# terra-render/Terra

Hardware: AMD Instinct MI355X
Metric: Msamples/s (higher is better)
Workload: dtype f32; 1 GPU; cornell_1080p_512spp; scene=cornell32, width=1920, height=1080, spp=512, bounces=8, integrator=simple, triangles=32, tree=auto, traversal=reference tree + leaf-box cull, tile=64, sample_split=8, parallelism=single

## Files before the change

include/terra_amd.h:

```cpp
#ifndef TERRA_AMD_H
#define TERRA_AMD_H

#include "Terra.h"

#ifdef __cplusplus
extern "C" {
#endif

typedef enum {
    kTerraAmdOk               = 0,
    kTerraAmdErrNoDevice      = -1,
    kTerraAmdErrNotCommitted  = -2,
    kTerraAmdErrUnsupported   = -3,
    kTerraAmdErrBadArgument   = -4,
    kTerraAmdErrLaunch        = -5
} TerraAmdStatus;

const char* terra_amd_last_error ( void );
void        terra_amd_clear_error ( void );
int         terra_amd_first_error ( char* buf, size_t capacity );
void        terra_amd_clear_first_error ( void );
size_t      terra_amd_thread_staging_bytes ( void );

int  terra_amd_init ( void );
// ... 403 lines not shown
int terra_amd_sh_irradiance ( const TerraAmdProbeSH* sh, size_t probes, const TerraAmdProbeGrid* grid, const TerraAmdPoint* points, const int* index, size_t n, float* out4 );
int terra_amd_probe_grid_points ( const TerraAmdProbeGrid* grid, TerraAmdPoint* out, int capacity );

#define kTerraAmdProbeVisibilityBackface 1
typedef struct {
    int   texels;
    int   sharpness;
    float max_distance;
    float bias;
    int   flags;
    int   reserved[3];
} TerraAmdProbeVisibility;
typedef struct {
    float weight;
    float distance;
    float distance2;
    int   cells;
} TerraAmdVisibilityTexel;
TERRA_ABI_ASSERT ( sizeof ( TerraAmdProbeVisibility ) == 32 );
TERRA_ABI_ASSERT ( offsetof ( TerraAmdProbeVisibility, sharpness ) == 4 );
TERRA_ABI_ASSERT ( offsetof ( TerraAmdProbeVisibility, max_distance ) == 8 );
TERRA_ABI_ASSERT ( offsetof ( TerraAmdProbeVisibility, bias ) == 12 );
TERRA_ABI_ASSERT ( offsetof ( TerraAmdProbeVisibility, flags ) == 16 );
TERRA_ABI_ASSERT ( offsetof ( TerraAmdProbeVisibility, reserved ) == 20 );
TERRA_ABI_ASSERT ( sizeof ( TerraAmdVisibilityTexel ) == 16 );
TERRA_ABI_ASSERT ( offsetof ( TerraAmdVisibilityTexel, distance ) == 4 );
TERRA_ABI_ASSERT ( offsetof ( TerraAmdVisibilityTexel, distance2 ) == 8 );
TERRA_ABI_ASSERT ( offsetof ( TerraAmdVisibilityTexel, cells ) == 12 );
int terra_amd_probe_visibility_device ( const void* d_hits, const void* d_rays, size_t probes, int cells, const TerraAmdProbeVisibility* options, int accumulate, void* d_map, void* stream );
int terra_amd_probe_visibility ( const TerraAmdHit* hits, const TerraAmdRay* rays, size_t probes_n, int cells, const TerraAmdProbeVisibility* options, int accumulate, TerraAmdVisibilityTexel* map );
int terra_amd_sh_irradiance_visible_device ( const void* d_sh, const void* d_map, size_t probes, const TerraAmdProbeGrid* grid, const TerraAmdProbeVisibility* options, const void* d_points, size_t n, void* d_out, void* stream );
int terra_amd_sh_irradiance_visible ( const TerraAmdProbeSH* sh, const TerraAmdVisibilityTexel* map, size_t probes, const TerraAmdProbeGrid* grid, const TerraAmdProbeVisibility* options, const TerraAmdPoint* points, size_t n, float* out4 );

int terra_amd_render_device_sharded ( const TerraCamera* camera, HTerraScene scene,
                                      void* d_pixels, void* d_results, size_t fb_width, size_t fb_height,
                                      size_t x, size_t y, size_t width, size_t height,
                                      size_t tile_size, int rank, int world,
                                      void* d_rand_calls, void* stream );

int    terra_amd_shard_tile_count ( size_t width, size_t height, size_t tile_size, int rank, int world );
size_t terra_amd_shard_packed_bytes ( size_t width, size_t height, size_t tile_size, int world );
int terra_amd_pack_tiles ( const void* d_pixels, const void* d_results, size_t fb_width, size_t fb_height,
                           size_t x, size_t y, size_t width, size_t height, size_t tile_size, int rank, int world,
                           void* d_packed, void* stream );
int terra_amd_unpack_tiles ( void* d_pixels, void* d_results, size_t fb_width, size_t fb_height,
                             size_t x, size_t y, size_t width, size_t height, size_t tile_size, int rank, int world,
                             const void* d_packed, void* stream );

int terra_amd_synchronize ( void* stream );

int terra_amd_time_render_device ( const TerraCamera* camera, HTerraScene scene,
                                   void* d_pixels, void* d_results, size_t fb_width, size_t fb_height,
                                   size_t x, size_t y, size_t width, size_t height,
                                   int launches, void* stream, float* ms_avg );


int terra_amd_unit_pcg ( const uint32_t* seeds, int nseeds, int n, float* out );
int terra_amd_unit_stream_keys ( uint64_t frame_seed, const uint64_t* pix, const uint64_t* samples_so_far, int n, uint64_t* out3 );
int terra_amd_unit_ray_aabb ( int n, const float* origins3, const float* dirs3, const float* boxes6, int* hit, float* tmin, float* tmax );
int terra_amd_unit_watertight ( int n, const float* origins3, const float* dirs3, const float* tris9, int* hit, float* out8 );
int terra_amd_unit_watertight_pair ( int n, const float* origins3, const float* dirs3, const float* quads12, int* hit2, float* depth2 );
int terra_amd_unit_moller_trumbore ( int n, const float* origins3, const float* dirs3, const float* tris9, int* hit, float* out4 );
int terra_amd_unit_bvh_traverse ( HTerraScene scene, int n, const float* origins3, const float* dirs3, int* found, uint32_t* prim, float* point3 );
int terra_amd_unit_bvh_traverse_fast ( HTerraScene scene, int n, const float* origins3, const float* dirs3, int* found, uint32_t* prim, float* point3, uint32_t* nodes_visited );
int terra_amd_unit_raycast ( HTerraScene scene, int n, const float* origins3, const float* dirs3, int* obj, int* tri, float* point3, float* surface47 );
int terra_amd_unit_trace ( HTerraScene scene, int n, const float* origins3, const float* dirs3, const uint64_t* stateB, const uint64_t* incB, float* radiance3, uint32_t* rand_calls );
int terra_amd_unit_bsdf ( int kind, int n, float* surfaces47, const float* e3, const float* wo3, float* wi3, float* pdf, float* f3 );
int terra_amd_unit_bsdf_at ( int kind, int n, const float* surfaces47, const float* wi3, const float* wo3, float* pdf, float* f3 );
int terra_amd_unit_camera ( const TerraCamera* camera, size_t fb_width, size_t fb_height, int n, const uint32_t* xy2, float jitter, const float* r2, float* dirs3 );
int terra_amd_unit_tonemap ( int op, float gamma, int n, float* colors3 );
int terra_amd_unit_math ( int fn, int n, const float* x, const float* y, float* out );
int terra_amd_scene_lds_plan ( HTerraScene scene, uint32_t* out6 );
int terra_amd_unit_exact_div ( int op, const float* a, const float* b, const float* c, uint64_t first, uint64_t count, float denominator, float reciprocal, uint64_t seed,
                               uint32_t* helper_bits, uint32_t* plain_bits, uint64_t* mismatches, uint32_t* first_bad );
int terra_amd_unit_exact_sqrt ( int op, const float* a, const float* b, const float* c, uint64_t first, uint64_t count, uint64_t seed,
                                uint32_t* helper_bits, uint32_t* plain_bits, uint64_t* mismatches, uint32_t* first_bad );
int terra_amd_unit_half_outward ( const double* x, int n, int up, uint16_t* out );
int terra_amd_unit_stratified ( const uint32_t* seeds, int nseeds, int strata, int samples_per_stratum, int n, float* out2 );
int terra_amd_unit_halton ( int first, int n, float* out2 );
int terra_amd_unit_distribution_1d ( const float* f, size_t n, const float* e, int m, float* x, float* pdf, uint32_t* idx, float* cdf_out, float* integral_out );
int terra_amd_unit_distribution_2d ( const float* f, size_t nx, size_t ny, const float* e12, int m, float* xy2, float* pdf, float* marginal_cdf_out );
int terra_amd_unit_distribution_2d_pdf ( const float* f, size_t nx, size_t ny, const float* xy2, int m, float* pdf );
int terra_amd_unit_azimuth24 ( uint32_t* mismatches );
int terra_amd_unit_texture_sample ( const TerraTexture* texture, int n, const float* uv2, float* out3 );
int terra_amd_unit_texture_latlong ( const TerraTexture* texture, int n, const float* dir3, float* out3 );

#ifdef __cplusplus
}
#endif
#endif
```

terra_amd/csrc/dev_types.h:

```cpp
#pragma once
#include <stdint.h>
#include <stddef.h>
#include <hip/hip_vector_types.h>

#define TERRA_DEV_MAX_ATTR 8

struct DevF3 { float x, y, z; };
struct DevF4 { float x, y, z, w; };

#define DEV_CHILD_LEAF  0x80000000u
#define DEV_CHILD_EMPTY 0xFFFFFFFFu

struct DevNode {
    float    min0[3], max0[3];
    float    min1[3], max1[3];
    uint32_t child[2];
    uint32_t prim[2];
};
static_assert ( sizeof ( DevNode ) == 64, "DevNode must be 64 bytes" );

struct DevFastNode {
    uint32_t q[3][2][4];
    uint32_t child[4];
    uint32_t pad[4];
// ... 104 lines not shown
#define TERRA_LEAF_CAP_RESIDENT_MIN 8
#endif
#ifndef TERRA_LDS_BLOCK_MAX_KB
#define TERRA_LDS_BLOCK_MAX_KB 156
#endif
#ifndef TERRA_JOB_ORDER_MIN_BLOCKS
#define TERRA_JOB_ORDER_MIN_BLOCKS 256
#endif

struct DevScene {
    const DevNode*     nodes;
    const DevTri*      tris;
    const DevProps*    props;
    const DevMaterial* mats;
    const DevLight*    lights;
    const float*       tri_area;
    const DevTexture*  textures;
    uint32_t n_nodes, n_tris, n_objects, n_lights;
    uint32_t lights_triangles_count;
    int32_t  max_stack;
    const DevNode*     fast_nodes;
    const DevFastNode* fast_nodes_h;
    const DevTri*      fast_tris;
    uint32_t n_fast_nodes;
    int32_t  fast_max_stack;
    float    fast_inv_scale;
    const struct DevReplay* ref_replay;
    const uint32_t*    fast_leaf_parent;
    const uint32_t*    fast_leaf_mask;
    uint32_t           reach;
    const float2*      sincos24;
    int32_t  env_mode;
    int32_t  env_tex;
    float    env_color[3];
    const float* env_f; const float* env_cdf; const float* env_row_f; const float* env_row_cdf;
    uint32_t env_nx, env_ny; float env_integral; uint32_t env_monotone;
};
#define TERRA_KIND_ENV 16
#define TERRA_KIND_TEX 32
#define TERRA_KIND_SAMPLER 64
#define TERRA_KIND_ENV_MIS 128

enum { kCtrRays = 0, kCtrNodes, kCtrBoxTests, kCtrTriTests, kCtrHits, kCtrSamples, kCtrRandCalls, kCtrAttrFetches, kCtrPixels, kCtrLaunches, kCtrFaults, kCtrTriCulled,
       kCtrDbg0, kCtrDbgLast = kCtrDbg0 + 15, kCtrSkipProved , kCtrCount };

struct DevRenderParams {
    DevScene scene;
    float    cam_rot[9];
    float    cam_pos[3];
    float    tan_half_fov;
    float    aspect;
    float    jitter;
    float    exposure;
    float    gamma;
    uint32_t fb_w, fb_h;
    uint32_t x, y, w, h;
    uint32_t st_x, st_y, st_pitch;
    uint32_t tile_size, rank, world;
    uint32_t spp;
    uint32_t split, split_log2, chunk_spp;
    float4*  partials;
    uint4*   job_streams;
    uint32_t job_blocks;
    uint32_t* job_queue;
    const uint32_t* block_order;
    uint32_t job_div_bpt2, job_div_tiles_x, job_div_bpt, job_tiles_x;
    uint32_t bounces;
    int32_t  integrator;
    int32_t  tonemap;
    uint64_t frame_seed;
    float*   pixels;
    void*    results;
    uint32_t* rand_calls;
    unsigned long long* counters;
    uint32_t stack_depth, leaf_cap, lds_nodes, lds_tris;
    uint32_t* stack_spill; uint32_t spill_cap;
    int32_t  lds_mode;
    int32_t  count_level;
    uint32_t bsdf_kinds;
    uint32_t leaf_cull;
    uint32_t fused_slab;
    uint32_t leaf_rank;
    uint32_t sampler_mode, sampler_strata;
    const uint32_t* job_live;
    const DevLeafBox* leaf_boxes;
    uint32_t n_leaf_boxes;
    uint32_t leaf_pairs;
    float    inv_fb_w, inv_fb_h;
};
struct DevLaunchMask { const uint32_t* words; uint32_t* live_blocks; };
#define TERRA_CLASS_MASKED 3u
struct DevRayRenderParams : DevRenderParams { const float4* rays; };
struct DevLens {
    int32_t model;
    float   lens_radius;
    float   focus_distance;
    float   ortho_half;
    float   fisheye_half;
};
struct DevLensRenderParams : DevRenderParams { DevLens lens; };
struct DevPointSampling {
    int32_t distribution;
};
struct DevPointRenderParams : DevRenderParams { const float4* points; DevPointSampling sampling; };
#ifndef TERRA_RAY_SOURCE
#if defined ( TERRA_TU ) && TERRA_TU >= 12
#define TERRA_RAY_SOURCE 3
#elif defined ( TERRA_TU ) && TERRA_TU >= 8
#define TERRA_RAY_SOURCE 2
#elif defined ( TERRA_TU ) && TERRA_TU >= 4
#define TERRA_RAY_SOURCE 1
#else
#define TERRA_RAY_SOURCE 0
#endif
#endif
```

terra_amd/csrc/exact_div.h:

```cpp
#pragma once
#include <hip/hip_runtime.h>
#include <stdint.h>

#define XD __device__ __forceinline__

XD int xd_in_range ( float v ) { const float a = __builtin_fabsf ( v ); return ( int ) ( a >= 0x1p-60f ) & ( int ) ( a <= 0x1p60f ); }
XD int xd_rcp_ok ( float d ) { return xd_in_range ( d ) & ( int ) ( ( __float_as_uint ( d ) & 0x7fffffu ) != 0x7fffffu ); }

XD float xd_rcp_short ( float d ) {
    float y = __builtin_amdgcn_rcpf ( d );
    float e = __builtin_fmaf ( -d, y, 1.f );
    y = __builtin_fmaf ( e, y, y );
    e = __builtin_fmaf ( -d, y, 1.f );
    return __builtin_fmaf ( e, y, y );
}
XD float xd_div_short ( float x, float d, float r ) {
    const float q0 = x * r;
    const float rem = __builtin_fmaf ( -d, q0, x );
    return __builtin_fmaf ( rem, r, q0 );
}
XD float xd_div_short_pos ( float x, float d, float r ) {
    const float q0 = x * r;
    const float nrem = __builtin_fmaf ( d, q0, -x );
    return __builtin_fmaf ( -nrem, r, q0 );
}

XD float rcp_exact ( float d ) {
    if ( xd_rcp_ok ( d ) ) return xd_rcp_short ( d );
    return 1.f / d;
}
XD float div_exact_r ( float x, float d, float r ) {
    if ( xd_in_range ( x ) & xd_in_range ( d ) ) return xd_div_short ( x, d, r );
    return x / d;
}
XD float div_exact_rk ( float x, float d, float r ) {
    if ( xd_in_range ( x ) ) return xd_div_short ( x, d, r );
    return x / d;
}
XD void div2_exact_rk ( float x1, float x2, float d1, float r1, float d2, float r2, float& q1, float& q2 ) {
    if ( xd_in_range ( x1 ) & xd_in_range ( x2 ) ) { q1 = xd_div_short ( x1, d1, r1 ); q2 = xd_div_short ( x2, d2, r2 ); return; }
    q1 = x1 / d1; q2 = x2 / d2;
}
XD void div2_exact ( float x1, float x2, float d, float& q1, float& q2 ) {
    if ( xd_rcp_ok ( d ) & xd_in_range ( x1 ) & xd_in_range ( x2 ) ) {
        const float r = xd_rcp_short ( d );
        q1 = xd_div_short ( x1, d, r ); q2 = xd_div_short ( x2, d, r );
        return;
    }
    q1 = x1 / d; q2 = x2 / d;
}
XD void rcp3_exact ( float dx, float dy, float dz, float& rx, float& ry, float& rz ) {
    if ( xd_rcp_ok ( dx ) & xd_rcp_ok ( dy ) & xd_rcp_ok ( dz ) ) { rx = xd_rcp_short ( dx ); ry = xd_rcp_short ( dy ); rz = xd_rcp_short ( dz ); return; }
    rx = 1.f / dx; ry = 1.f / dy; rz = 1.f / dz;
}
XD int xd_component_ok ( float c ) { return ( int ) ( c == 0.f ) | ( int ) ( __builtin_fabsf ( c ) >= 0x1p-60f ); }
XD void xd_normalize3 ( float x, float y, float z, float l, float& qx, float& qy, float& qz ) {
    if ( ( int ) ( l >= 0x1p-60f ) & ( int ) ( l <= 0x1p60f ) & ( int ) ( ( __float_as_uint ( l ) & 0x7fffffu ) != 0x7fffffu ) & xd_component_ok ( x ) & xd_component_ok ( y ) & xd_component_ok ( z ) ) {
        const float r = xd_rcp_short ( l );
        qx = xd_div_short_pos ( x, l, r ); qy = xd_div_short_pos ( y, l, r ); qz = xd_div_short_pos ( z, l, r );
        return;
    }
    qx = x / l; qy = y / l; qz = z / l;
}

XD float roulette_scale ( float pr ) {
    const double d = ( double ) pr + 1e-4;
    if ( ( int ) ( pr >= 0.f ) & ( int ) ( pr <= 0x1p60f ) ) {
        double y = __builtin_amdgcn_rcp ( d );
        double e = __builtin_fma ( -d, y, 1.0 ); y = __builtin_fma ( y, e, y );
        e = __builtin_fma ( -d, y, 1.0 ); y = __builtin_fma ( y, e, y );
        e = __builtin_fma ( -d, y, 1.0 ); y = __builtin_fma ( e, y, y );
        return ( float ) y;
    }
    return ( float ) ( 1.0 / d );
}
```

terra_amd/csrc/exact_sqrt.h:

```cpp
#pragma once
#include <hip/hip_runtime.h>
#include <stdint.h>
#include "exact_div.h"

XD float xs_sqrt_short ( float x ) {
    const float s = __builtin_amdgcn_sqrtf ( x );
    const float down = __uint_as_float ( __float_as_uint ( s ) - 1u ), up = __uint_as_float ( __float_as_uint ( s ) + 1u );
    const float r_down = __builtin_fmaf ( -down, s, x ), r_up = __builtin_fmaf ( -up, s, x );
    float r = r_down <= 0.f ? down : s;
    r = r_up > 0.f ? up : r;
    return r;
}
XD int xs_in_range ( float x ) { return ( int ) ( x >= 0x1p-96f ) & ( int ) ( x <= 0x1.fffffep127f ); }
XD float sqrt_exact ( float x ) {
    if ( xs_in_range ( x ) ) return xs_sqrt_short ( x );
    return sqrtf ( x );
}
```

terra_amd/csrc/integrators_device.h:

```cpp
#pragma once
#include "shading_device.h"

TD float randf ( Pcg32& b, Counters& c, int count ) { if ( count == 2 ) ++c.rand_calls; return trng_b_float ( b ); }
TD uint32_t randf_bits ( Pcg32& b, Counters& c, int count ) { if ( count == 2 ) ++c.rand_calls; return trng_b_bits ( b ); }

TD float triangle_area ( V3 a, V3 b, V3 cc ) { return length ( cross ( b - a, cc - a ) ) / 2; }

struct LightSample { uint32_t light_object; uint32_t tri_in_object; uint32_t tri; float pick_pdf; V3 pos, norm; };

template <int COUNT, int MODE = 0>
TD LightSample draw_light_sample ( const DevScene& sc, Pcg32& rb, Counters& c, const Tracer* T = nullptr ) {
    LightSample ls;
    float e = ( float ) ( ( double ) randf ( rb, c, COUNT ) - 1e-4 );
    double xl = ( double ) e * ( double ) sc.n_lights;
    uint32_t li = xl < 0 ? 0u : ( uint32_t ) xl;
    ls.pick_pdf = 1.f / ( float ) sc.lights_triangles_count;
    DevLight l = ( MODE == 1 && T ) ? T->l_lights[li] : sc.lights[li];
    float e_t = randf ( rb, c, COUNT );
    uint32_t k = ( uint32_t ) ( e_t * ( float ) l.tri_count );
    if ( k >= l.tri_count ) k = l.tri_count - 1;
    ls.light_object = l.object; ls.tri_in_object = k; ls.tri = l.first_tri + k;
    float e1 = randf ( rb, c, COUNT ), e2 = randf ( rb, c, COUNT );
    const float4* tris = ( MODE == 1 && T ) ? reinterpret_cast<const float4*> ( T->l_tris ) : reinterpret_cast<const float4*> ( sc.tris );
    const float4* props = ( MODE == 1 && T ) ? T->l_props : reinterpret_cast<const float4*> ( sc.props );
// ... 236 lines not shown
                    L = L * ( dot ( wi, sf.normal ) * weight / bpdf );
                    Lo = Lo + L;
                }
            }
        }
        if constexpr ( ( KINDS & TERRA_KIND_ENV_MIS ) != 0 && !DEBUG_WEIGHTS ) {
            if ( !h.hit && bpdf > 0.f ) {
                uint32_t col, row; float st;
                environment_texel ( sc, wi, col, row, st );
                const float epdf = ( !bsdf_is_singular<KINDS> ( sf ) && dot ( wi, sf.normal ) > 0 ) ? environment_texel_pdf ( sc, col, row, st ) : 0.f;
                const float r = epdf / bpdf, weight = 1.f / ( 1.f + r * r );
                V3 L = had ( texture_read ( sc.textures[sc.env_tex], col, row ), f );
                L = L * ( dot ( wi, sf.normal ) * weight / bpdf );
                Lo = Lo + L;
            }
        }
    }
    if constexpr ( ( KINDS & TERRA_KIND_SAMPLER ) != 0 && !DEBUG_WEIGHTS ) { if ( env_sampling_active ( sc ) ) Lo = Lo + environment_light_sample<COUNT, MODE, KINDS, true> ( T, sf, p, wo, rb, c ); }
    return had ( Lo, throughput );
}

TD V3 integrate_debug_normals ( const Surface& sf, uint32_t bounce ) {
    if ( bounce != 0 ) return v3 ( 0, 0, 0 );
    V3 n = sf.normal;
    V3 pp = v3 ( sel_min ( n.x > 0 ? n.x : 0.f, 1.f ), sel_min ( n.y > 0 ? n.y : 0.f, 1.f ), sel_min ( n.z > 0 ? n.z : 0.f, 1.f ) );
    V3 nn = v3 ( sel_min ( n.x > -1 ? n.x : -1.f, 0.f ), sel_min ( n.y > -1 ? n.y : -1.f, 0.f ), sel_min ( n.z > -1 ? n.z : -1.f, 0.f ) );
    nn = nn * -1.f;
    V3 col = v3 ( 0, 0, 0 );
    col = col + v3 ( 1, 0, 0 ) * pp.x;
    col = col + v3 ( 0, 1, 0 ) * pp.y;
    col = col + v3 ( 0, 0, 1 ) * pp.z;
    col = col + v3 ( 0, 1, 1 ) * nn.x;
    col = col + v3 ( 1, 0, 1 ) * nn.y;
    col = col + v3 ( 1, 1, 0 ) * nn.z;
    return col;
}

template <int INTEGRATOR, int COUNT, int MODE, int KINDS>
TD V3 integrate ( const Tracer& T, const Ray& ray, Surface& sf, V3 p, V3 wo, V3 throughput, uint32_t bounce, Pcg32& rb, Counters& c ) {
    if ( INTEGRATOR == 0 ) {
        if ( dot ( wo, sf.normal ) > 0 ) return had ( sf.emissive, throughput );
        return v3 ( 0, 0, 0 );
    } else if ( INTEGRATOR == 1 ) {
        return integrate_direct<COUNT, MODE, KINDS> ( T, sf, p, wo, throughput, bounce, rb, c );
    } else if ( INTEGRATOR == 2 ) {
        return integrate_mis<COUNT, MODE, KINDS, false> ( T, sf, p, wo, throughput, bounce, rb, c );
    } else if ( INTEGRATOR == 3 ) {
        return bounce != 0 ? v3 ( 0, 0, 0 ) : v3 ( 1, 1, 1 );
    } else if ( INTEGRATOR == 4 ) {
        if ( bounce != 0 ) return v3 ( 0, 0, 0 );
        float d = length ( ray.o - p ) / 500.f;
        return v3 ( d, d, d );
    } else if ( INTEGRATOR == 5 ) {
        return integrate_debug_normals ( sf, bounce );
    } else {
        return integrate_mis<COUNT, MODE, KINDS, true> ( T, sf, p, wo, throughput, bounce, rb, c );
    }
}

template <int COUNT>
TD PathDraws path_draw ( const float2* sincos24, Pcg32& rb, Counters& c ) {
    PathDraws d;
    d.e0 = randf ( rb, c, COUNT );
    const uint32_t k1 = randf_bits ( rb, c, COUNT );
    d.e1 = trng_b_from_bits ( k1 );
    d.e2 = randf ( rb, c, COUNT );
    d.az = azimuth_fetch_index ( sincos24, k1 );
    d.e3 = randf ( rb, c, COUNT );
    return d;
}
template <int KINDS>
TD bool path_continue ( Surface& sf, V3 wo, V3& throughput, uint32_t& bounce, uint32_t max_bounces, const PathDraws& d, V3& wi ) {
    wi = bsdf_sample<KINDS> ( sf, d.e0, d.e1, d.e2, wo, d.az );
    float pdf = sel_max ( bsdf_pdf<KINDS> ( sf, wi, wo ), ( float ) 1e-4 );
    V3 f = bsdf_eval<KINDS> ( sf, wi, wo ) * rcp_exact ( pdf );
    throughput = had ( throughput, f );
    throughput = throughput * dot ( sf.normal, wi );
    float pr = sel_max ( throughput.x, sel_max ( throughput.y, throughput.z ) );
    if ( d.e3 > pr ) return false;
        throughput = throughput * roulette_scale ( pr );
    ++bounce;
    return bounce <= max_bounces;
}
struct SamplerPair { float u0, u1; bool on; };
TD SamplerPair sampler_pair_none() { SamplerPair s; s.u0 = s.u1 = 0.f; s.on = false; return s; }
TD void path_apply_sampler ( PathDraws& d, const SamplerPair& sp, uint32_t bounce ) {
    if ( sp.on && bounce == 0 ) { d.e0 = sp.u0; d.e1 = sp.u1; d.az = azimuth_none(); }
}
TD SamplerPair sampler_pair_draw ( uint32_t mode, uint32_t strata, uint64_t n, Pcg32& stream_a ) {
    SamplerPair s = sampler_pair_none();
    if ( mode == 1 ) { s.u0 = radical_inverse ( 3, n ); s.u1 = radical_inverse ( 2, n ); s.on = true; }
    else if ( mode == 2 && strata > 0 ) {
        const uint64_t cap = ( uint64_t ) strata * strata * 16ull, m = n % cap, stratum = m / 16ull;
        const float stratum_size = 1.f / ( float ) strata;
        s.u0 = sd_below_one ( ( ( float ) ( uint32_t ) ( stratum % strata ) + trng_a_float ( stream_a ) ) * stratum_size );
        s.u1 = sd_below_one ( ( ( float ) ( uint32_t ) ( stratum / strata ) + trng_a_float ( stream_a ) ) * stratum_size );
        s.on = true;
    }
    return s;
}
template <int COUNT, int KINDS>
TD bool path_continue ( const DevScene& sc, Surface& sf, V3 wo, V3& throughput, uint32_t& bounce, uint32_t max_bounces, Pcg32& rb, Counters& c, V3& wi, const SamplerPair& sp = sampler_pair_none() ) {
    PathDraws d = path_draw<COUNT> ( sc.sincos24, rb, c );
    if ( KINDS & TERRA_KIND_SAMPLER ) path_apply_sampler ( d, sp, bounce );
    return path_continue<KINDS> ( sf, wo, throughput, bounce, max_bounces, d, wi );
}

template <int INTEGRATOR, int COUNT, int MODE, int KINDS>
TD V3 trace_path ( const Tracer& T, Ray ray, uint32_t bounces, Pcg32& rb, Counters& c ) {
    V3 Lo = v3 ( 0, 0, 0 ), throughput = v3 ( 1, 1, 1 );
    for ( uint32_t bounce = 0; bounce <= bounces; ++bounce ) {
        Surface sf;
        RaycastResult h = scene_raycast<COUNT, MODE, KINDS> ( T, ray, sf, c );
        if ( !h.hit ) {
            if ( ( KINDS & TERRA_KIND_ENV ) && T.sc.env_mode && !env_reaches_by_samples<INTEGRATOR, KINDS> ( T.sc, bounce ) ) { throughput = had ( throughput, environment_eval ( T.sc, ray.d ) ); Lo = Lo + throughput; }
            break;
        }
        V3 wo = neg ( ray.d );
        Lo = Lo + integrate<INTEGRATOR, COUNT, MODE, KINDS> ( T, ray, sf, h.point, wo, throughput, bounce, rb, c );
        V3 wi;
        uint32_t next_bounce = bounce;
        if ( !path_continue<COUNT, KINDS> ( T.sc, sf, wo, throughput, next_bounce, bounces, rb, c, wi ) ) break;
        ray = surface_ray ( sf, h.point, wi );
    }
    return Lo;
}

TD V3 uncharted2 ( V3 x ) {
    const float A = 0.15f, B = 0.5f, C = 0.1f, D = 0.2f, E = 0.02f, F = 0.3f;
    V3 r;
    r.x = ( ( x.x * ( A * x.x + C * B ) + D * E ) / ( x.x * ( A * x.x + B ) + D * F ) ) - E / F;
    r.y = ( ( x.y * ( A * x.y + C * B ) + D * E ) / ( x.y * ( A * x.y + B ) + D * F ) ) - E / F;
    r.z = ( ( x.z * ( A * x.z + C * B ) + D * E ) / ( x.z * ( A * x.z + B ) + D * F ) ) - E / F;
    return r;
}
TD V3 powv ( V3 c, float e ) { return v3 ( tdm_powf ( c.x, e ), tdm_powf ( c.y, e ), tdm_powf ( c.z, e ) ); }
TD V3 tonemap ( V3 c, int op, float gamma ) {
    switch ( op ) {
        case 1: c = powv ( c, 1.f / gamma ); break;
        case 2:
            c.x = c.x / ( 1.f + c.x ); c.y = c.y / ( 1.f + c.y ); c.z = c.z / ( 1.f + c.z );
            c = powv ( c, 1.f / gamma ); break;
        case 3: {
            V3 x = v3 ( sel_max ( 0.f, c.x - 0.004f ), sel_max ( 0.f, c.y - 0.004f ), sel_max ( 0.f, c.z - 0.004f ) );
            c.x = ( x.x * ( 6.2f * x.x + 0.5f ) ) / ( x.x * ( 6.2f * x.x + 1.7f ) + 0.06f );
            c.y = ( x.y * ( 6.2f * x.y + 0.5f ) ) / ( x.y * ( 6.2f * x.y + 1.7f ) + 0.06f );
            c.x = ( x.z * ( 6.2f * x.z + 0.5f ) ) / ( x.z * ( 6.2f * x.z + 1.7f ) + 0.06f );
            break;
        }
        case 4: {
            V3 ws = uncharted2 ( v3 ( 11.2f, 11.2f, 11.2f ) );
            ws = v3 ( 1.f / ws.x, 1.f / ws.y, 1.f / ws.z );
            V3 t = uncharted2 ( c * 2.f );
            c = powv ( had ( t, ws ), 1.f / gamma );
            break;
        }
        default: break;
    }
    return c;
}
```

terra_amd/csrc/kernels.h:

```cpp
#pragma once
#include <hip/hip_runtime.h>
#include "dev_types.h"

hipError_t terra_launch_render ( const DevRenderParams& p, hipStream_t stream );
hipError_t terra_launch_job_streams ( const DevRenderParams& p, hipStream_t stream );
hipError_t terra_launch_block_order ( const DevRenderParams& p, uint32_t* cls, hipStream_t stream, const DevLaunchMask* mask, bool classify, bool prove );
hipError_t terra_launch_render_mode0 ( const DevRenderParams& p, size_t lds, hipStream_t stream );
hipError_t terra_launch_render_mode1 ( const DevRenderParams& p, size_t lds, hipStream_t stream );
hipError_t terra_launch_render_mode2 ( const DevRenderParams& p, size_t lds, hipStream_t stream );
hipError_t terra_launch_render_mode3 ( const DevRenderParams& p, size_t lds, hipStream_t stream );
hipError_t terra_launch_render_rays ( const DevRenderParams& p, const void* rays, hipStream_t stream );
hipError_t terra_launch_render_rays_mode0 ( const DevRayRenderParams& p, size_t lds, hipStream_t stream );
hipError_t terra_launch_render_rays_mode1 ( const DevRayRenderParams& p, size_t lds, hipStream_t stream );
hipError_t terra_launch_render_rays_mode2 ( const DevRayRenderParams& p, size_t lds, hipStream_t stream );
hipError_t terra_launch_render_rays_mode3 ( const DevRayRenderParams& p, size_t lds, hipStream_t stream );
hipError_t terra_launch_render_lens ( const DevRenderParams& p, const DevLens& lens, hipStream_t stream );
hipError_t terra_launch_render_lens_mode0 ( const DevLensRenderParams& p, size_t lds, hipStream_t stream );
hipError_t terra_launch_render_lens_mode1 ( const DevLensRenderParams& p, size_t lds, hipStream_t stream );
hipError_t terra_launch_render_lens_mode2 ( const DevLensRenderParams& p, size_t lds, hipStream_t stream );
hipError_t terra_launch_render_lens_mode3 ( const DevLensRenderParams& p, size_t lds, hipStream_t stream );
hipError_t terra_launch_render_points ( const DevRenderParams& p, const void* points, const DevPointSampling& sampling, hipStream_t stream );
hipError_t terra_launch_render_points_mode0 ( const DevPointRenderParams& p, size_t lds, hipStream_t stream );
hipError_t terra_launch_render_points_mode1 ( const DevPointRenderParams& p, size_t lds, hipStream_t stream );
hipError_t terra_launch_render_points_mode2 ( const DevPointRenderParams& p, size_t lds, hipStream_t stream );
hipError_t terra_launch_render_points_mode3 ( const DevPointRenderParams& p, size_t lds, hipStream_t stream );
hipError_t terra_launch_resolve ( const DevRenderParams& p, hipStream_t stream, const uint32_t* live_blocks );
hipError_t terra_launch_tiles ( bool pack, float* pixels, void* results, uint32_t fb_w, uint32_t x, uint32_t y, uint32_t w, uint32_t h,
                                uint32_t tile, uint32_t rank, uint32_t world, float* packed, hipStream_t stream );

hipError_t terra_launch_aov ( DevRenderParams p, void* aov, hipStream_t stream, const uint32_t* mask );
hipError_t terra_launch_aov_rays ( DevRenderParams p, const void* rays, void* aov, hipStream_t stream );
hipError_t terra_launch_aov_lens ( DevRenderParams p, const DevLens& lens, void* aov, hipStream_t stream );
hipError_t terra_launch_aov_points ( DevRenderParams p, const void* points, const DevPointSampling& sampling, void* aov, hipStream_t stream );

hipError_t terra_launch_denoise ( const void* results, const void* aov, uint32_t fb_w, uint32_t x, uint32_t y, uint32_t w, uint32_t h, int iterations,
                                  float exposure, int op, float gamma, float* radiance, float* pixels, hipStream_t stream );
hipError_t terra_launch_denoise_variance ( const void* results, const void* aov, const void* moments, uint32_t fb_w, uint32_t x, uint32_t y, uint32_t w, uint32_t h, int iterations,
                                           float exposure, int op, float gamma, float* radiance, float* pixels, hipStream_t stream );

hipError_t terra_launch_moments_accumulate ( const void* results, void* moments, uint32_t fb_w, uint32_t x, uint32_t y, uint32_t w, uint32_t h, hipStream_t stream );
hipError_t terra_launch_tile_error ( const void* moments, uint32_t fb_w, uint32_t x, uint32_t y, uint32_t w, uint32_t h, uint32_t tile, float* errors, hipStream_t stream );
hipError_t terra_launch_error_mask ( const float* errors, uint32_t w, uint32_t h, uint32_t tile, float target, int all, uint32_t* mask, hipStream_t stream );

struct DevTemporalParams {
    float cam_pos[3], cam_rot[9], tan_half_fov, aspect;
    float prev_pos[3], prev_rot[9], prev_tan_half_fov;
    uint32_t fb_w, fb_h, x, y, w, h;
    float alpha, depth_tolerance, normal_cos, max_length;
    uint32_t same_camera;
    float inv_fb_w, inv_fb_h;
};
hipError_t terra_launch_temporal_reproject ( const DevTemporalParams& p, const void* results, const void* aov, const void* history_in, void* history_out,
                                             void* out_results, void* out_moments, hipStream_t stream );

struct DevQueryParams {
    DevScene scene;
    uint32_t fast, stack_depth, leaf_cap, spill_cap, leaf_cull;
    float    origin_limit;
};
hipError_t terra_launch_query ( DevQueryParams p, const void* rays, size_t n, void* out, bool anyhit, hipStream_t stream );

struct DevAtlas {
    uint32_t width, height;
    float    uv_scale[2], uv_offset[2], margin;
};
hipError_t terra_launch_atlas_points ( const DevScene& sc, const DevAtlas& atlas, const float* uvs, void* points, void* texels, hipStream_t stream );
hipError_t terra_launch_dilate ( float* data, int channels, int* valid, uint32_t width, uint32_t height, int passes, hipStream_t stream );

struct DevProbeGrid {
    int32_t on;
    int32_t count[3];
    float   origin[3], spacing[3];
};
hipError_t terra_launch_probe_rays ( const void* probes, uint32_t count, uint32_t cells, const float* jitter, void* rays, hipStream_t stream );
hipError_t terra_launch_sh_project ( const void* results, const void* rays, uint32_t count, uint32_t cells, int batch, void* sh, hipStream_t stream );
hipError_t terra_launch_sh_irradiance ( const void* sh, uint32_t probes, const DevProbeGrid& grid, const void* points, const int* index, uint32_t n, void* out, hipStream_t stream );
struct DevProbeVisibility {
    int32_t texels, sharpness;
    float   max_distance, bias;
    int32_t backface;
};
hipError_t terra_launch_probe_visibility ( const void* hits, const void* rays, uint32_t count, uint32_t cells, const DevProbeVisibility& options, int accumulate, void* map, hipStream_t stream );
hipError_t terra_launch_sh_irradiance_visible ( const void* sh, const void* map, const DevProbeGrid& grid, const DevProbeVisibility& options, const void* points, uint32_t n, void* out, hipStream_t stream );

hipError_t terra_fill_sincos24 ( float2* table, hipStream_t stream );
hipError_t terra_unit_azimuth24 ( const float2* table, float2* computed, uint32_t* mismatches );

hipError_t terra_unit_pcg ( const uint32_t* seeds, int nseeds, int n, float* out );
hipError_t terra_unit_stream_keys ( uint64_t frame_seed, const uint64_t* pix, const uint64_t* k, int n, uint64_t* out3 );
hipError_t terra_unit_ray_aabb ( int n, const float* o, const float* d, const float* boxes, int* hit, float* tmin, float* tmax );
hipError_t terra_unit_watertight ( int n, const float* o, const float* d, const float* tris, int* hit, float* out8 );
hipError_t terra_unit_watertight_pair ( int n, const float* o, const float* d, const float* quads, int* hit, float* depth );
hipError_t terra_unit_moller_trumbore ( int n, const float* o, const float* d, const float* tris, int* hit, float* out4 );
hipError_t terra_unit_bvh_traverse ( const DevScene& sc, int n, const float* o, const float* d, int* found, uint32_t* prim, float* point );
hipError_t terra_unit_bvh_traverse_fast ( const DevScene& sc, int n, const float* o, const float* d, int* found, uint32_t* prim, float* point, uint32_t* nodes_visited );
hipError_t terra_unit_raycast ( const DevScene& sc, int n, const float* o, const float* d, int* obj, int* tri, float* point, float* surface47 );
hipError_t terra_unit_trace ( const DevScene& sc, int integrator, uint32_t bounces, int n, const float* o, const float* d,
                              const uint64_t* stateB, const uint64_t* incB, float* radiance, uint32_t* rand_calls );
hipError_t terra_unit_bsdf ( int kind, int n, float* surfaces47, const float* e3, const float* wo3, float* wi3, float* pdf, float* f3 );
hipError_t terra_unit_bsdf_at ( int kind, int n, const float* surfaces47, const float* wi3, const float* wo3, float* pdf, float* f3 );
hipError_t terra_unit_camera ( const DevRenderParams& p, int n, const uint32_t* xy2, const float* r2, float* dirs3 );
hipError_t terra_unit_lens_rays ( const DevRenderParams& p, const DevLens& lens, int n, const uint32_t* xy2, const float* r4, float* rays8 );
hipError_t terra_unit_point_rays ( const DevPointSampling& sampling, int n, const float* points8, const float* g2, float* rays8 );
hipError_t terra_unit_tonemap ( int op, float gamma, int n, float* colors3 );
hipError_t terra_unit_math ( int fn, int n, const float* x, const float* y, float* out );
hipError_t terra_unit_exact_div ( int op, const float* a, const float* b, const float* c, uint64_t first, uint64_t count, float D, float R, uint64_t seed,
                                  uint32_t* helper_bits, uint32_t* plain_bits, unsigned long long* mismatches, uint32_t* first_bad );
hipError_t terra_unit_exact_sqrt ( int op, const float* a, const float* b, const float* c, uint64_t first, uint64_t count, uint64_t seed,
                                   uint32_t* helper_bits, uint32_t* plain_bits, unsigned long long* mismatches, uint32_t* first_bad );
hipError_t terra_unit_texture_sample ( const DevTexture* t, int n, const float* uv2, float* out3 );
hipError_t terra_unit_texture_latlong ( const DevTexture* t, int n, const float* dir3, float* out3 );
hipError_t terra_unit_stratified ( const uint32_t* seeds, int nseeds, int strata, int samples, int n, float* out2 );
hipError_t terra_unit_halton ( int first, int n, float* out2 );
hipError_t terra_unit_distribution_1d ( const float* f, uint32_t n, float* cdf, float* integral, uint32_t* monotone, const float* e, int m, float* x, float* pdf, uint32_t* idx );
hipError_t terra_unit_distribution_2d ( const float* f, uint32_t nx, uint32_t ny, float* cdf, float* integrals, float* mcdf, uint32_t* monotone, const float* e12, int m, float* xy2, float* pdf );
hipError_t terra_unit_distribution_2d_pdf ( const float* f, uint32_t nx, uint32_t ny, float* cdf, float* integrals, float* mcdf, uint32_t* monotone, const float* xy2, int m, float* pdf );
hipError_t terra_build_fast_tree_device ( const DevTri* tris, const uint32_t* rank, uint32_t n, float extra_margin, DevNode* out_nodes, DevTri* out_tris, uint32_t* n_nodes_out, int* max_stack_out, hipStream_t stream );
```

terra_amd/csrc/render_kernels.hip:

```cpp
#include <hip/hip_runtime.h>
#include "trace_device.h"
#include "kernels.h"
#include "launch_plan.h"
#include "empty_proof.h"

#ifdef TERRA_TU
#define TERRA_TU_HAS(k) ( TERRA_TU == ( k ) )
#define TERRA_TU_MODE(k) ( TERRA_TU == ( k ) || TERRA_TU == ( k ) + 4 || TERRA_TU == ( k ) + 8 || TERRA_TU == ( k ) + 12 )
#else
#define TERRA_TU_HAS(k) ( !TERRA_RAY_SOURCE )
#define TERRA_TU_MODE(k) 1
#endif
#if TERRA_RAY_SOURCE == 3
typedef DevPointRenderParams RenderKernelParams;
#elif TERRA_RAY_SOURCE == 2
typedef DevLensRenderParams RenderKernelParams;
#elif TERRA_RAY_SOURCE == 1
typedef DevRayRenderParams RenderKernelParams;
#else
typedef DevRenderParams RenderKernelParams;
#endif

struct DevResult { float acc[3]; int samples; };

// ... 322 lines not shown
        p.partials[ ( ( size_t ) chunk * ( p.job_blocks >> p.split_log2 ) + blk ) * 256 + ( fin & 255u )] = make_float4 ( aux[0], aux[256], aux[512], __uint_as_float ( COUNT == 2 ? c.rand_calls - auxu[1024] : 0u ) );
        auxu[768] = TERRA_JOB_NONE;
    }
    PoolWord* pool = job_pool_of_wave ( aux );
    const unsigned long long m = __ballot ( 1 );
    const uint32_t lane = threadIdx.x & 63u, n = ( uint32_t ) __popcll ( m ), ahead = ( uint32_t ) __popcll ( m & ( ( 1ull << lane ) - 1ull ) );
    uint32_t next = pool_load ( pool ), end = pool_load ( pool + 1 );
    const uint32_t take = n < end - next ? n : end - next;
    uint32_t job = next + ahead;
    bool got = ahead < take;
    next += take;
    if ( take < n && next < total && p.job_queue ) {
        uint32_t base = 0;
        if ( ahead == 0 ) base = atomicAdd ( p.job_queue, TERRA_JOB_BATCH );
        base = ( uint32_t ) __builtin_amdgcn_readfirstlane ( ( int ) base );
        next = base < total ? base : total; end = base + TERRA_JOB_BATCH < total ? base + TERRA_JOB_BATCH : total;
        const uint32_t take2 = n - take < end - next ? n - take : end - next;
        if ( !got ) { job = next + ( ahead - take ); got = ahead - take < take2; }
        next += take2;
    }
    if ( ahead == 0 ) { pool_store ( pool, next ); pool_store ( pool + 1, end ); }
    if ( !got ) { j.exhausted = true; return; }
    uint32_t chunk;
    int prior_samples;
    if constexpr ( TABLE ) {
        const uint4 e1 = p.job_streams[2 * ( size_t ) job + 1];
        const uint4 e0 = p.job_streams[2 * ( size_t ) job];
        asm volatile ( "" : : "v" ( e0.x ), "v" ( e0.y ), "v" ( e0.z ), "v" ( e0.w ), "v" ( e1.x ), "v" ( e1.y ), "v" ( e1.z ), "v" ( e1.w ) );
        if ( e1.z == 0xffffffffu ) return;
        j.px = e1.z & 0xffffu; j.py = e1.z >> 16;
        chunk = ( job >> 8 ) & ( p.split - 1 );
        rs.a.state = ( uint64_t ) e0.x | ( ( uint64_t ) e0.y << 32 ); rs.a.inc = 1;
        rs.b.state = ( uint64_t ) e0.z | ( ( uint64_t ) e0.w << 32 ); rs.b.inc = ( uint64_t ) e1.x | ( ( uint64_t ) e1.y << 32 );
        rs.seedA = 0;
        prior_samples = ( int ) e1.w;
    } else {
        if ( !job_pixel ( p, job, j.px, j.py, chunk ) ) return;
        prior_samples = reinterpret_cast<const DevResult*> ( p.results ) [ ( size_t ) ( j.py - p.st_y ) * p.st_pitch + ( j.px - p.st_x )].samples;
        rs = trng_pixel_streams ( p.frame_seed, ( uint64_t ) j.py * p.fb_w + j.px, ( uint64_t ) ( uint32_t ) prior_samples + ( uint64_t ) chunk * p.chunk_spp );
    }
    aux[0] = 0.f; aux[256] = 0.f; aux[512] = 0.f; auxu[768] = job;
    if ( COUNT == 2 ) auxu[1024] = c.rand_calls;
    j.s = 0; j.base = ( uint32_t ) prior_samples + chunk * p.chunk_spp;
}

#ifndef TERRA_RAY_HOLD
#define TERRA_RAY_HOLD 0
#endif
struct PrimaryRay { V3 o, d; };
TD PrimaryRay ray_record ( const RenderKernelParams& p, uint32_t px, uint32_t py ) {
    PrimaryRay r; r.o = v3 ( 0, 0, 0 ); r.d = v3 ( 0, 0, 1 );
#if TERRA_RAY_SOURCE == 1
    const float4* rec = p.rays + 2 * ( ( size_t ) ( py - p.st_y ) * p.st_pitch + ( px - p.st_x ) );
    const float4 q0 = rec[0], q1 = rec[1];
    r.o = v3 ( q0.x, q0.y, q0.z ); r.d = v3 ( q1.x, q1.y, q1.z );
#elif TERRA_RAY_SOURCE == 3
    const float4* rec = p.points + 2 * ( ( size_t ) ( py - p.st_y ) * p.st_pitch + ( px - p.st_x ) );
    const float4 q0 = rec[0], q1 = rec[1];
    r.o = v3 ( q0.x, q0.y, q0.z ); r.d = v3 ( q1.x, q1.y, q1.z );
#endif
    return r;
}
TD bool ray_record_inactive ( const PrimaryRay& r ) {
    const bool finite = fabsf ( r.o.x ) < INFINITY && fabsf ( r.o.y ) < INFINITY && fabsf ( r.o.z ) < INFINITY && fabsf ( r.d.x ) < INFINITY && fabsf ( r.d.y ) < INFINITY && fabsf ( r.d.z ) < INFINITY;
    return !finite || ( r.d.x == 0.f && r.d.y == 0.f && r.d.z == 0.f );
}
#ifndef TERRA_POINT_HOLD
#define TERRA_POINT_HOLD 0
#endif
#if TERRA_RAY_SOURCE == 3
#define TERRA_PRIMARY_RAY( ro, rd, r1, r2 )
#define TERRA_LENS_RAY( ro, rd, r1, r2 ) do { const PrimaryRay pt_ = TERRA_POINT_HOLD ? held : ray_record ( p, jb.px, jb.py ); const float g1_ = trng_a_float ( rs.a ), g2_ = trng_a_float ( rs.a ); point_sample ( p.sampling, pt_.o, pt_.d, g1_, g2_, ro, rd ); } while ( 0 )
#define TERRA_JOB_NEXT() job_take<COUNT, MODE == 1> ( p, acc_lds, jb, rs, c, job_total, held )
#elif TERRA_RAY_SOURCE == 2
#define TERRA_PRIMARY_RAY( ro, rd, r1, r2 )
#define TERRA_LENS_RAY( ro, rd, r1, r2 ) do { float l1_ = 0.f, l2_ = 0.f; if ( lens_draws ( p.lens ) ) { l1_ = trng_a_float ( rs.a ); l2_ = trng_a_float ( rs.a ); } lens_sample ( p, p.lens, jb.px, jb.py, r1, r2, l1_, l2_, ro, rd ); } while ( 0 )
#define TERRA_JOB_NEXT() job_next<COUNT, MODE == 1> ( p, acc_lds, jb, rs, c, job_total )
#elif TERRA_RAY_SOURCE == 1
#define TERRA_PRIMARY_RAY( ro, rd, r1, r2 ) do { const PrimaryRay pr_ = TERRA_RAY_HOLD ? held : ray_record ( p, jb.px, jb.py ); ro = pr_.o; rd = pr_.d; } while ( 0 )
#define TERRA_LENS_RAY( ro, rd, r1, r2 )
#define TERRA_JOB_NEXT() job_take<COUNT, MODE == 1> ( p, acc_lds, jb, rs, c, job_total, held )
#else
#define TERRA_LENS_RAY( ro, rd, r1, r2 )
#define TERRA_PRIMARY_RAY( ro, rd, r1, r2 ) ro = cam_pos; rd = camera_sample ( p, jb.px, jb.py, r1, r2 )
#define TERRA_JOB_NEXT() job_next<COUNT, MODE == 1> ( p, acc_lds, jb, rs, c, job_total )
#endif
#if TERRA_RAY_SOURCE == 1 || TERRA_RAY_SOURCE == 3
template <int COUNT, bool TABLE>
TD void job_take ( const RenderKernelParams& p, float* aux, Jobs& j, PixelStreams& rs, const Counters& c, uint32_t total, PrimaryRay& held ) {
    job_next<COUNT, TABLE> ( p, aux, j, rs, c, total );
    if ( j.s != p.chunk_spp ) {
        const PrimaryRay r = ray_record ( p, j.px, j.py );
#if TERRA_RAY_SOURCE == 3
        if ( point_inactive ( r.o, r.d ) ) j.s = p.chunk_spp;
        if ( TERRA_POINT_HOLD ) held = r;
#else
        if ( ray_record_inactive ( r ) ) j.s = p.chunk_spp;
        if ( TERRA_RAY_HOLD ) held = r;
#endif
    }
}
#endif

template <int INTEGRATOR, int COUNT, int MODE, int KINDS>
__global__ __launch_bounds__ ( 256, terra_waves ( INTEGRATOR, KINDS, MODE ) ) void terra_render_kernel ( RenderKernelParams p ) {
    extern __shared__ float4 lds_f4[];
    const int tid = threadIdx.x;
    Tracer T0 = make_tracer<MODE> ( p.scene, lds_f4, p.stack_depth, p.leaf_cap, p.lds_nodes, p.lds_tris, p.leaf_cull != 0, p.fused_slab != 0, p.leaf_rank != 0, p.leaf_boxes, p.n_leaf_boxes, terra_leaf_pair_table ( p ) );
    if constexpr ( MODE == 1 && COUNT == 0 ) T0.nearest = T0.pairs && T0.n_boxes != 0u && ( p.leaf_pairs & TERRA_LEAF_PAIRS_NEAREST ) != 0u;
    T0.faults = p.counters + kCtrFaults;
    if ( MODE >= 2 && p.stack_spill ) { T0.spill = p.stack_spill + ( size_t ) ( blockIdx.x * 256u + threadIdx.x ) * p.spill_cap; T0.spill_cap = p.spill_cap; }
    const Tracer T = T0;

    PixelStreams rs = trng_pixel_streams ( 0, 0, 0 );
    Counters c = counters_zero();
    float* acc_lds = reinterpret_cast<float*> ( T.stack - tid ) + ( p.stack_depth + p.leaf_cap ) * TERRA_COL + tid;
    uint32_t job_total = p.job_blocks * 256u;
    if constexpr ( MODE == 1 ) { if ( p.job_live ) job_total = *p.job_live; }
    job_init_lane ( p, acc_lds );
    Jobs jb; jb.px = jb.py = 0; jb.s = p.chunk_spp; jb.exhausted = false; jb.base = 0;
    SamplerPair sp = sampler_pair_none();
    V3 Lo = v3 ( 0, 0, 0 ), throughput = v3 ( 1, 1, 1 );
    Ray ray = make_ray ( v3 ( 0, 0, 0 ), v3 ( 0, 0, 1 ) );
    uint32_t bounce = 0;
    const V3 cam_pos = v3p ( p.cam_pos );
#if TERRA_RAY_SOURCE == 1 || TERRA_RAY_SOURCE == 3
    PrimaryRay held; held.o = v3 ( 0, 0, 0 ); held.d = v3 ( 0, 0, 1 );
#endif

    if constexpr ( terra_decoupled_mis ( INTEGRATOR, MODE, KINDS ) ) {
        LaneTraversal lt = lane_traversal_idle ( T, ray );
        int job = 0;
        bool done = false, have_ray = false, cont = false;
        MisPending pend; pend.a_vis = pend.a_hid = pend.f2 = pend.p = pend.t_before = v3 ( 0, 0, 0 ); pend.expected = 0; pend.bpdf2 = pend.cos2 = 0.f; pend.light_object = 0;
        V3 cont_o = v3 ( 0, 0, 0 ), cont_d = v3 ( 0, 0, 1 ), b_o = v3 ( 0, 0, 0 ), b_d = v3 ( 0, 0, 1 ), lo_i = v3 ( 0, 0, 0 );
        for ( ;; ) {
            if ( !lt.traversing && !done && ! ( have_ray && lane_traversal_recheck<MODE> ( T, ray, lt ) ) ) {
                bool start = false;
                V3 ro = v3 ( 0, 0, 0 ), rd = v3 ( 0, 0, 1 );
                if ( have_ray && job != 0 ) {
                    Ray r = ray; r.o = r.o + r.d * 0.001f;
                    const bool hit = lt.best.tri != 0xffffffffu;
                    Surface lsf; uint32_t object = 0, tri_in_object = 0, nattr = 0, tri_s = 0xffffffffu;
                    V3 point = hit ? r.o + r.d * lt.best.depth : v3 ( FLT_MAX, FLT_MAX, FLT_MAX );
                    if ( hit ) {
                        if ( job == 2 ) { surface_init<MODE, KINDS> ( T, lt.best.tri, point, lsf, object, tri_in_object, nattr ); tri_s = MODE >= 2 ? T.sc.mats[object].first_tri + tri_in_object : lt.best.tri; }
                        else { tri_s = hit_soup_index<MODE> ( T, lt.best.tri ); const float4 t0 = reinterpret_cast<const float4*> ( T.sc.tris ) [3 * tri_s]; object = __float_as_uint ( t0.w ); nattr = T.sc.mats[object].attributes_count; }
                        if ( COUNT ) ++c.hits;
                        if ( COUNT == 2 ) c.attr_fetches += nattr + 1;
                    }
                    if ( job == 1 ) {
                        lo_i = tri_s == pend.expected ? pend.a_vis : pend.a_hid;
                        ro = b_o; rd = b_d; job = 2; start = true;
                    } else {
                        Lo = Lo + mis_finish_b<MODE> ( T, pend, lo_i, hit, object, tri_s, point, lsf, ray.d );
                        job = 0;
                        if ( cont ) { ro = cont_o; rd = cont_d; start = true; }
                        else { deposit ( acc_lds, Lo ); have_ray = false; }
                    }
                } else if ( have_ray ) {
                    if ( lt.best.tri != 0xffffffffu ) {
                        Surface sf;
                        V3 point = shade_surface<COUNT, MODE, KINDS> ( T, ray, lt.best, sf, c );
                        V3 wo = neg ( ray.d );
                        Ray ray_a;
                        pend = mis_prepare<COUNT, KINDS, MODE> ( T, sf, point, wo, throughput, bounce, rs.b, c, ray_a, b_d );
                        b_o = surface_origin ( sf, point );
// ... 57 lines not shown
                    if ( jb.s == p.chunk_spp ) { TERRA_JOB_NEXT(); if ( jb.exhausted ) done = true; }
                    if ( jb.s != p.chunk_spp ) {
                        float r1 = trng_a_float ( rs.a ), r2 = trng_a_float ( rs.a );
                        TERRA_PRIMARY_RAY ( ro, rd, r1, r2 );
                        if constexpr ( ( KINDS & TERRA_KIND_SAMPLER ) != 0 ) sp = sampler_pair_draw ( p.sampler_mode, p.sampler_strata, ( uint64_t ) jb.base + jb.s, rs.a );
                        TERRA_LENS_RAY ( ro, rd, r1, r2 );
                        Lo = v3 ( 0, 0, 0 ); throughput = v3 ( 1, 1, 1 ); bounce = 0; ++jb.s; start = true;
                    }
                }
                if ( start ) {
                    ray = make_ray ( ro, rd ); lane_traversal_start<COUNT, MODE> ( T, ray, lt, c ); have_ray = true;
                    if ( shadow ) lane_traversal_expect<COUNT, MODE> ( T, ray, lt, pend.expected );
                }
            }
            if ( !lane_traversal_run<COUNT, MODE> ( T, ray, lt, c ) && __all ( done ) ) break;
        }
    } else if constexpr ( terra_decoupled ( INTEGRATOR, MODE ) ) {
        LaneTraversal lt = lane_traversal_idle ( T, ray );
        bool done = false, have_ray = false;
        for ( ;; ) {
            if ( !lt.traversing && !done && ! ( have_ray && lane_traversal_recheck<MODE> ( T, ray, lt ) ) ) {
                bool next = false;
                V3 ro = v3 ( 0, 0, 0 ), rd = v3 ( 0, 0, 1 );
                if ( have_ray ) {
                    if ( lt.best.tri != 0xffffffffu ) {
                        Surface sf;
                        PathDraws pd = path_draw<COUNT> ( azimuth_table<MODE> ( T.sc ), rs.b, c );
                        if constexpr ( ( KINDS & TERRA_KIND_SAMPLER ) != 0 ) path_apply_sampler ( pd, sp, bounce );
                        V3 point = shade_surface<COUNT, MODE, KINDS> ( T, ray, lt.best, sf, c );
                        V3 wo = neg ( ray.d ), wi;
                        Lo = Lo + integrate<INTEGRATOR, COUNT, MODE, KINDS> ( T, ray, sf, point, wo, throughput, bounce, rs.b, c );
                        next = path_continue<KINDS> ( sf, wo, throughput, bounce, p.bounces, pd, wi );
                        if ( next ) { ro = surface_origin ( sf, point ); rd = wi; }
                    } else if ( ( KINDS & TERRA_KIND_ENV ) && T.sc.env_mode ) {
                        throughput = had ( throughput, environment_eval ( T.sc, ray.d ) );
                        Lo = Lo + throughput;
                    }
                    if ( !next ) { deposit ( acc_lds, Lo ); have_ray = false; }
                }
                if ( !next ) {
                    if ( jb.s == p.chunk_spp ) { TERRA_JOB_NEXT(); if ( jb.exhausted ) done = true; }
                    if ( jb.s != p.chunk_spp ) {
                        float r1 = trng_a_float ( rs.a ), r2 = trng_a_float ( rs.a );
                        TERRA_PRIMARY_RAY ( ro, rd, r1, r2 );
                        if constexpr ( ( KINDS & TERRA_KIND_SAMPLER ) != 0 ) sp = sampler_pair_draw ( p.sampler_mode, p.sampler_strata, ( uint64_t ) jb.base + jb.s, rs.a );
                        TERRA_LENS_RAY ( ro, rd, r1, r2 );
                        Lo = v3 ( 0, 0, 0 ); throughput = v3 ( 1, 1, 1 ); bounce = 0; ++jb.s; next = true;
                    }
                }
                if ( next ) { ray = make_ray ( ro, rd ); lane_traversal_start<COUNT, MODE> ( T, ray, lt, c ); have_ray = true; }
            }
            if ( !lane_traversal_run<COUNT, MODE> ( T, ray, lt, c ) && __all ( done ) ) break;
        }
    } else {
    bool alive = false;
    V3 ro = v3 ( 0, 0, 0 ), rd = v3 ( 0, 0, 1 );
    constexpr bool LO_LDS = MODE == 1;
    float* lo_lds = acc_lds + 6 * 256;
    auto lo_reset = [&] () { if ( LO_LDS ) { lo_lds[0] = 0.f; lo_lds[256] = 0.f; lo_lds[512] = 0.f; } else Lo = v3 ( 0, 0, 0 ); };
    auto lo_add = [&] ( V3 t ) {
        if ( LO_LDS ) { if ( t.x != 0.f || t.y != 0.f || t.z != 0.f ) { lo_lds[0] = lo_lds[0] + t.x; lo_lds[256] = lo_lds[256] + t.y; lo_lds[512] = lo_lds[512] + t.z; } }
        else Lo = Lo + t;
    };
    auto lo_deposit = [&] () { if ( LO_LDS ) deposit ( acc_lds, v3 ( lo_lds[0], lo_lds[256], lo_lds[512] ) ); else deposit ( acc_lds, Lo ); };
#ifndef TERRA_REGEN_MIN
#define TERRA_REGEN_MIN 1
#endif
    while ( true ) {
        const bool any_alive = __any ( alive );
        if ( !alive && ( TERRA_REGEN_MIN <= 1 || !any_alive || __popcll ( __ballot ( !alive ) ) >= TERRA_REGEN_MIN ) ) {
            if ( jb.s == p.chunk_spp && ( TERRA_JOB_FETCH_MIN <= 1 || !any_alive || __popcll ( __ballot ( jb.s == p.chunk_spp ) ) >= TERRA_JOB_FETCH_MIN ) ) TERRA_JOB_NEXT();
            if ( jb.exhausted ) break;
            if ( jb.s != p.chunk_spp ) {
                PS_WAVE ( c, kPsCamIter ); PS_LANE ( c, kPsCamLanes );
                float r1 = trng_a_float ( rs.a ), r2 = trng_a_float ( rs.a );
                TERRA_PRIMARY_RAY ( ro, rd, r1, r2 );
                if constexpr ( ( KINDS & TERRA_KIND_SAMPLER ) != 0 ) sp = sampler_pair_draw ( p.sampler_mode, p.sampler_strata, ( uint64_t ) jb.base + jb.s, rs.a );
                TERRA_LENS_RAY ( ro, rd, r1, r2 );
                lo_reset(); throughput = v3 ( 1, 1, 1 ); bounce = 0; alive = true; ++jb.s;
            }
        }
        if ( alive ) {
            bool guarded = false;
            if constexpr ( ray_start_masks_for ( COUNT, MODE, KINDS ) ) ray = make_ray_guarded ( ro, rd, guarded ); else
            ray = make_ray ( ro, rd );
            Surface sf;
            PS_WAVE ( c, kPsRayIter ); PS_LANE ( c, kPsRayLanes );
            constexpr bool pre_draw = !TERRA_IS_LIGHT ( INTEGRATOR );
            PathDraws pd;
            RaycastResult h = scene_raycast<COUNT, MODE, KINDS> ( T, ray, sf, c, pre_draw ? &pd : nullptr, pre_draw ? &rs.b : nullptr, guarded );
            bool end = !h.hit;
            if ( h.hit ) {
                PS_WAVE ( c, kPsShadeIter ); PS_LANE ( c, kPsShadeLanes );
                V3 wo = neg ( ray.d ), wi;
                constexpr bool SPLIT_DIRECT = INTEGRATOR == 1 && ( KINDS & ( TERRA_KIND_TEX | TERRA_KIND_SAMPLER ) ) == 0;
                if constexpr ( SPLIT_DIRECT ) {
                    Ray shadow_ray;
                    const DirectPending pend = direct_prepare<COUNT, KINDS, MODE> ( T, sf, h.point, wo, throughput, bounce, rs.b, c, shadow_ray );
                    pd = path_draw<COUNT> ( azimuth_table<MODE> ( T.sc ), rs.b, c );
                    end = !path_continue<KINDS> ( sf, wo, throughput, bounce, p.bounces, pd, wi );
                    if ( !end ) { ro = surface_origin ( sf, h.point ); rd = wi; }
                    const uint32_t tri = scene_raycast_triangle<COUNT, MODE, ray_start_masks_for ( COUNT, MODE, KINDS )> ( T, shadow_ray, c, pend.expected );
                    lo_add ( tri == pend.expected ? pend.vis : pend.hid );
                } else if constexpr ( INTEGRATOR == 2 && ( KINDS & ( TERRA_KIND_TEX | TERRA_KIND_SAMPLER ) ) == 0 ) {
                    Ray ray_a; V3 b_d;
                    const MisPending pend = mis_prepare<COUNT, KINDS, MODE> ( T, sf, h.point, wo, throughput, bounce, rs.b, c, ray_a, b_d );
                    const V3 next_o = surface_origin ( sf, h.point );
                    end = !path_continue<COUNT, KINDS> ( T.sc, sf, wo, throughput, bounce, p.bounces, rs.b, c, wi, sp );
                    if ( !end ) { ro = next_o; rd = wi; }
                    const uint32_t tri_a = scene_raycast_triangle<COUNT, MODE, ray_start_masks_for ( COUNT, MODE, KINDS )> ( T, ray_a, c, pend.expected );
                    const V3 lo_a = tri_a == pend.expected ? pend.a_vis : pend.a_hid;
                    Surface lsf;
                    const RaycastResult hb = scene_raycast<COUNT, MODE, KINDS> ( T, make_ray ( next_o, b_d ), lsf, c );
                    lo_add ( mis_finish_b<MODE> ( T, pend, lo_a, hb.hit, hb.object, hb.tri, hb.point, lsf, b_d ) );
                } else {
                lo_add ( integrate<INTEGRATOR, COUNT, MODE, KINDS> ( T, ray, sf, h.point, wo, throughput, bounce, rs.b, c ) );
                if ( !pre_draw ) pd = path_draw<COUNT> ( azimuth_table<MODE> ( T.sc ), rs.b, c );
                if constexpr ( ( KINDS & TERRA_KIND_SAMPLER ) != 0 ) path_apply_sampler ( pd, sp, bounce );
                end = !path_continue<KINDS> ( sf, wo, throughput, bounce, p.bounces, pd, wi );
                if ( !end ) { ro = surface_origin ( sf, h.point ); rd = wi; }
                }
            } else if ( ( KINDS & TERRA_KIND_ENV ) && T.sc.env_mode && !env_reaches_by_samples<INTEGRATOR, KINDS> ( T.sc, bounce ) ) {
                throughput = had ( throughput, environment_eval ( T.sc, ray.d ) );
                lo_add ( throughput );
            }
            if ( end ) { lo_deposit(); alive = false; }
        }
    }
    }

    if ( COUNT ) wave_flush_counters ( c, p.counters );
    if ( COUNT == 2 && p.leaf_cull ) {
        unsigned long long x = c.tri_culled;
        for ( int off = 32; off > 0; off >>= 1 ) x += __shfl_xor ( x, off, 64 );
        if ( ( threadIdx.x & 63 ) == 0 && x ) atomicAdd ( &p.counters[kCtrTriCulled], x );
    }
#if TERRA_PHASE_STATS
    for ( int k = 0; k < 16; ++k ) {
        unsigned long long x = c.ps[k];
        for ( int off = 32; off > 0; off >>= 1 ) x += __shfl_xor ( x, off, 64 );
        if ( ( threadIdx.x & 63 ) == 0 && x ) atomicAdd ( &p.counters[kCtrDbg0 + k], x );
    }
#endif
}


static uint32_t resident_blocks ( const void* fn, size_t lds ) {
    struct Key { const void* fn; size_t lds; int dev; uint32_t blocks; };
    static thread_local Key cache[8]; static thread_local int used = 0;
    int dev = 0; ( void ) hipGetDevice ( &dev );
    for ( int i = 0; i < used; ++i ) if ( cache[i].fn == fn && cache[i].lds == lds && cache[i].dev == dev ) return cache[i].blocks;
    int per_cu = 0;
    if ( hipOccupancyMaxActiveBlocksPerMultiprocessor ( &per_cu, fn, 256, lds ) != hipSuccess || per_cu < 1 ) { ( void ) hipGetLastError(); per_cu = 1; }
    const uint32_t blocks = ( uint32_t ) per_cu * terra_cu_count();
    Key& k = cache[used < 8 ? used++ : 7]; k.fn = fn; k.lds = lds; k.dev = dev; k.blocks = blocks;
    return blocks;
}
template <int I, int COUNT, int MODE, int KINDS>
static hipError_t launch_instance ( const RenderKernelParams& p, size_t lds, hipStream_t stream ) {
    auto fn = terra_render_kernel<I, COUNT, MODE, KINDS>;
    if ( lds > ( size_t ) 64 * 1024 ) {
        if ( lds > terra_lds_block_limit() ) return hipErrorInvalidValue;
        static thread_local size_t opted[8] = { 0 }; int dev = 0; ( void ) hipGetDevice ( &dev );
        if ( opted[dev & 7] < lds ) {
            const hipError_t e = hipFuncSetAttribute ( reinterpret_cast<const void*> ( fn ), hipFuncAttributeMaxDynamicSharedMemorySize, ( int ) lds );
            if ( e != hipSuccess ) return e;
            opted[dev & 7] = lds;
        }
    }
    uint32_t grid = p.job_blocks;
    if ( p.job_queue ) { const uint32_t cap = resident_blocks ( reinterpret_cast<const void*> ( fn ), lds ); if ( grid > cap ) grid = cap; }
    if ( MODE >= 2 && p.spill_cap && ( !p.stack_spill || terra_spill_bytes ( grid, p.spill_cap ) > terra_fast_spill_bytes ( p ) ) ) return hipErrorInvalidValue;
    hipLaunchKernelGGL ( fn, dim3 ( grid ), dim3 ( 256 ), lds, stream, p );
    return hipGetLastError();
}
template <int I, int MODE, int KINDS>
static hipError_t launch_kinds ( const RenderKernelParams& p, size_t lds, hipStream_t stream ) {
    if ( p.count_level == 0 ) return launch_instance<I, 0, MODE, KINDS> ( p, lds, stream );
    return launch_instance<I, 2, MODE, KINDS> ( p, lds, stream );
}
template <int I, int MODE>
static hipError_t launch_mode ( const RenderKernelParams& p, size_t lds, hipStream_t stream ) {
    if ( p.bsdf_kinds == 1 ) return launch_kinds<I, MODE, 1> ( p, lds, stream );
    if ( ( p.bsdf_kinds & ~3u ) == 0 ) return launch_kinds<I, MODE, 3> ( p, lds, stream );
    if constexpr ( I <= 2 && MODE != 0 ) {
        if ( ( p.bsdf_kinds & ~15u ) == 0 ) return launch_kinds<I, MODE, 15> ( p, lds, stream );
    }
    if ( ( p.bsdf_kinds & TERRA_KIND_SAMPLER ) == 0 ) return launch_kinds<I, MODE, TERRA_KINDS_ALL & ~TERRA_KIND_SAMPLER> ( p, lds, stream );
    if constexpr ( I == 2 ) {
        if ( p.bsdf_kinds & TERRA_KIND_ENV_MIS ) return launch_kinds<I, MODE, TERRA_KINDS_ALL | TERRA_KIND_ENV_MIS> ( p, lds, stream );
    }
    return launch_kinds<I, MODE, TERRA_KINDS_ALL> ( p, lds, stream );
}
template <int MODE>
static hipError_t launch_integrator ( const RenderKernelParams& p, size_t lds, hipStream_t stream ) {
    switch ( p.integrator ) {
        case 0: return launch_mode<0, MODE> ( p, lds, stream );
        case 1: return launch_mode<1, MODE> ( p, lds, stream );
        case 2: return launch_mode<2, MODE> ( p, lds, stream );
        case 3: return launch_mode<3, MODE> ( p, lds, stream );
        case 4: return launch_mode<4, MODE> ( p, lds, stream );
// ... 251 lines not shown
```

terra_amd/csrc/scene_host.cpp:

```cpp
#include <hip/hip_runtime.h>
#include <algorithm>
#include <cfloat>
#include <cmath>
#include <cstdarg>
#include <cstdio>
#include <cstdlib>
#include <cstring>
#include <mutex>
#include <string>
#include <unordered_set>
#include <atomic>
#include <chrono>
#include <vector>

#include "../../include/terra_amd.h"
#include "../../include/TerraPresets.h"
#include "dev_types.h"
#include "kernels.h"
#include "launch_plan.h"
#include "empty_proof.h"
#include "tree_build.h"
#include "multi_gpu.h"

static thread_local std::string g_last_error;
// ... 1240 lines not shown
    out6[3] = ( uint32_t ) TERRA_LDS_BUDGET; out6[4] = p.lds_mode == 1 ? p.lds_tris : 0u; out6[5] = p.leaf_rank;
    return 0;
}
extern "C" int terra_amd_leaf_pair_offsets ( uint32_t n, uint32_t* entries, uint32_t* planes ) {
    if ( n > TERRA_LEAF_RANK_MAX / 2 ) return fail ( kTerraAmdErrBadArgument, "terra_amd_leaf_pair_offsets: a pair section has at most %u entries", ( unsigned ) TERRA_LEAF_RANK_MAX / 2 );
    for ( uint32_t perm = 0; perm < 6u && entries; ++perm ) for ( uint32_t e = 0; e < n; ++e ) entries[perm * n + e] = terra_pair_entry_offset ( n, perm, e );
    for ( uint32_t k = 0; k < n && planes; ++k ) for ( uint32_t as = 0; as < 6u; ++as ) planes[6u * k + as] = terra_pair_boxes_offset ( n ) + terra_pair_box_plane_offset ( k, as >> 1, as & 1u );
    return ( int ) terra_pair_section_bytes ( n );
}
extern "C" int terra_amd_leaf_box_offsets ( uint32_t n, uint32_t* planes, uint32_t* masks ) {
    if ( n > TERRA_LEAF_RANK_MAX ) return fail ( kTerraAmdErrBadArgument, "terra_amd_leaf_box_offsets: a table has at most %u boxes", ( unsigned ) TERRA_LEAF_RANK_MAX );
    for ( uint32_t k = 0; k < n; ++k ) {
        for ( uint32_t as = 0; as < 6u && planes; ++as ) planes[6u * k + as] = terra_leaf_box_plane_offset ( k, as >> 1, as & 1u );
        if ( masks ) masks[k] = terra_leaf_box_mask_offset ( k );
    }
    return n ? ( int ) ( terra_leaf_box_plane_offset ( n - 1u, 0, 0 ) - terra_leaf_box_plane_offset ( 0, 0, 0 ) ) : 0;
}
static int sum_counters ( Scene* s, size_t first, size_t n, unsigned long long* out ) {
    unsigned long long c[kCtrCount];
    std::fill ( out, out + n, 0ull );
    for ( size_t k = s->replicas.size(); k-- > 0; ) {
        const Scene::Replica& r = s->replicas[k];
        HIP_TRY ( hipSetDevice ( r.device ), kTerraAmdErrNoDevice );
        HIP_TRY ( hipMemcpy ( c, r.d_counters + first, n * sizeof ( unsigned long long ), hipMemcpyDeviceToHost ), kTerraAmdErrNoDevice );
        for ( size_t i = 0; i < n; ++i ) out[i] += c[i];
    }
    return 0;
}
extern "C" int terra_amd_get_stats ( HTerraScene h, TerraAmdStats* out ) {
    Scene* s = S ( h );
    memset ( out, 0, sizeof *out );
    if ( !s->device_ok ) return fail ( kTerraAmdErrNotCommitted, "scene has no device replica" );
    unsigned long long c[kCtrCount];
    if ( int rc = sum_counters ( s, 0, kCtrCount, c ) ) return rc;
    out->rays = c[kCtrRays]; out->nodes = c[kCtrNodes]; out->tri_tests = c[kCtrTriTests]; out->hits = c[kCtrHits];
    out->rand_calls = c[kCtrRandCalls]; out->attr_fetches = c[kCtrAttrFetches]; out->tri_culled = c[kCtrTriCulled];
    out->box_tests = primary ( s ).dev.n_tris >= 2 ? ( s->tree.use_fast ? 4 * out->nodes : s->tree.cull_ok ? 2 * out->nodes : 2 * out->nodes - out->tri_tests ) : 0;
    out->samples = s->stat_samples; out->pixels = s->stat_pixels; out->launches = s->launches;
    return 0;
}
extern "C" long long terra_amd_debug_faults ( HTerraScene h ) {
    Scene* s = S ( h );
    unsigned long long v = 0;
    if ( !s->device_ok || sum_counters ( s, kCtrFaults, 1, &v ) ) return -1;
    return ( long long ) v;
}
extern "C" int terra_amd_debug_counters ( HTerraScene h, unsigned long long* out16 ) {
    Scene* s = S ( h );
    if ( !s->device_ok || !out16 ) return fail ( kTerraAmdErrNotCommitted, "scene has no device replica" );
    return sum_counters ( s, kCtrDbg0, 16, out16 );
}
extern "C" int terra_amd_reset_stats ( HTerraScene h ) {
    Scene* s = S ( h );
    if ( !s->device_ok ) return fail ( kTerraAmdErrNotCommitted, "scene has no device replica" );
    for ( size_t k = s->replicas.size(); k-- > 0; ) {
        HIP_TRY ( hipSetDevice ( s->replicas[k].device ), kTerraAmdErrNoDevice );
        HIP_TRY ( hipMemset ( s->replicas[k].d_counters, 0, kCtrCount * sizeof ( unsigned long long ) ), kTerraAmdErrNoDevice );
    }
    s->launches = 0; s->stat_pixels = 0; s->stat_samples = 0;
    return 0;
}

static uint32_t effective_spp ( const TerraSceneOptions& o ) {
    size_t spp = o.samples_per_pixel;
    if ( o.sampling_method == kTerraSamplingMethodStratified ) {
        size_t cur = o.strata * o.strata;
        while ( spp > cur && cur > 1 ) cur *= cur;
        if ( cur >= spp ) spp = cur;
    }
    return ( uint32_t ) spp;
}

static void fill_camera ( const TerraCamera* cam, size_t fb_w, size_t fb_h, DevRenderParams& p ) {
    TerraFloat3 z = terra_normf3 ( &cam->direction );
    TerraFloat3 xa = terra_crossf3 ( &cam->up, &z ); xa = terra_normf3 ( &xa );
    TerraFloat3 ya = terra_crossf3 ( &z, &xa );
    p.cam_rot[0] = xa.x; p.cam_rot[1] = ya.x; p.cam_rot[2] = z.x;
    p.cam_rot[3] = xa.y; p.cam_rot[4] = ya.y; p.cam_rot[5] = z.y;
    p.cam_rot[6] = xa.z; p.cam_rot[7] = ya.z; p.cam_rot[8] = z.z;
    p.cam_pos[0] = cam->position.x; p.cam_pos[1] = cam->position.y; p.cam_pos[2] = cam->position.z;
    p.tan_half_fov = ( float ) tan ( ( double ) ( ( cam->fov * 0.0174533f ) / 2 ) );
    p.aspect = ( float ) fb_w / ( float ) fb_h;
    p.inv_fb_w = 1.f / ( float ) fb_w; p.inv_fb_h = 1.f / ( float ) fb_h;
}

static int scene_check ( const Scene* s ) {
    if ( !s->committed ) return fail ( kTerraAmdErrNotCommitted, "terra_scene_commit has not run since the scene changed" );
    if ( !s->device_ok ) return fail ( kTerraAmdErrNoDevice, "scene has no device replica: %s", s->commit_error.c_str() );
    return 0;
}
static void apply_stack_hooks ( const Scene* s, DevRenderParams& p ) {
    if ( s->test_fast_stack_lds > 0 && p.lds_mode == 2 ) {
        const uint32_t need = p.stack_depth + p.spill_cap;
        p.stack_depth = need < ( uint32_t ) s->test_fast_stack_lds ? need : ( uint32_t ) s->test_fast_stack_lds; p.spill_cap = need - p.stack_depth;
    }
    if ( s->test_pad_stack > 0 && p.lds_mode != 1 ) {
        p.stack_depth += ( uint32_t ) s->test_pad_stack;
        p.leaf_cap = terra_clamp_leaf_cap ( p.stack_depth, p.leaf_cap, terra_lds_bytes ( p ) - ( size_t ) ( p.stack_depth + p.leaf_cap ) * 1024 );
    }
}
static int fill_params ( Scene* s, const Scene::Replica& r, const TerraCamera* cam, size_t fb_w, size_t fb_h, size_t x, size_t y, size_t w, size_t h,
                         size_t tile, int rank, int world, DevRenderParams& p, const bool* ray_origins_ok = nullptr ) {
    if ( int rc = scene_check ( s ) ) return rc;
    if ( ( !cam && !ray_origins_ok ) || w == 0 || h == 0 || x + w > fb_w || y + h > fb_h ) return fail ( kTerraAmdErrBadArgument, "bad tile rectangle %zu,%zu %zux%zu in %zux%zu", x, y, w, h, fb_w, fb_h );
    if ( tile == 0 || tile % 16 != 0 ) return fail ( kTerraAmdErrBadArgument, "tile_size %zu must be a positive multiple of 16", tile );
    if ( world < 1 || rank < 0 || rank >= world ) return fail ( kTerraAmdErrBadArgument, "bad shard %d/%d", rank, world );
    memset ( &p, 0, sizeof p );
    p.scene = r.dev;
    if ( cam ) fill_camera ( cam, fb_w, fb_h, p );
    p.jitter = s->opts.subpixel_jitter; p.exposure = s->opts.manual_exposure; p.gamma = s->opts.gamma;
    p.fb_w = ( uint32_t ) fb_w; p.fb_h = ( uint32_t ) fb_h;
    p.x = ( uint32_t ) x; p.y = ( uint32_t ) y; p.w = ( uint32_t ) w; p.h = ( uint32_t ) h;
    p.tile_size = ( uint32_t ) tile; p.rank = ( uint32_t ) rank; p.world = ( uint32_t ) world;
    p.st_x = 0; p.st_y = 0; p.st_pitch = ( uint32_t ) fb_w;
    p.spp = effective_spp ( s->opts );
    p.split = 1; p.split_log2 = 0; p.chunk_spp = p.spp; p.partials = nullptr; p.job_blocks = 0; p.job_queue = nullptr;
    p.bounces = ( uint32_t ) s->opts.bounces;
    p.integrator = ( int32_t ) s->opts.integrator; p.tonemap = ( int32_t ) s->opts.tonemapping_operator;
    if ( p.integrator < 0 || p.integrator > 6 ) return fail ( kTerraAmdErrBadArgument, "unknown integrator %d", p.integrator );
    if ( ( p.integrator == kTerraIntegratorDirect || p.integrator == kTerraIntegratorDirectMis || p.integrator == kTerraIntegratorDebugMisWeights ) && s->lights.empty() )
        return fail ( kTerraAmdErrBadArgument, "integrator %d needs at least one emissive object (the reference asserts, src/Terra.c:1617)", p.integrator );
    p.frame_seed = s->frame_seed;
    p.counters = r.d_counters;
    terra_plan_lds ( p );
    const TreeChoice& c = s->tree;
    const bool cam_ok = ray_origins_ok ? *ray_origins_ok : ( c.reach || c.reach_cull ) ? ( fabsf ( p.cam_pos[0] ) <= c.reach_limit && fabsf ( p.cam_pos[1] ) <= c.reach_limit && fabsf ( p.cam_pos[2] ) <= c.reach_limit ) : coords_within_margin ( p.cam_pos, 3 );
    if ( c.use_fast && r.dev.fast_nodes_h && ( s->tree_mode == 1 || cam_ok ) ) terra_plan_fast_tree ( p );
    else if ( ( c.use_fast || c.cull_ok ) && !cam_ok && !ray_origins_ok && !s->warned_camera.exchange ( true ) )
        fprintf ( stderr, "[terra_amd] warning: camera at (%g, %g, %g) lies outside the range (+-%g) for which this scene's traversal shortcut is proven: this call runs the reference "
                  "tree's replica traversal (same image, typically 10-20 x slower on large scenes); terra_amd_traversal_info() reports camera_limit and last_call\n",
                  ( double ) p.cam_pos[0], ( double ) p.cam_pos[1], ( double ) p.cam_pos[2], ( double ) shortcut_limit ( c ) );
    apply_stack_hooks ( s, p );
    p.leaf_cull = ( c.cull_ok && cam_ok && p.lds_mode != 2 ) ? 1u : 0u;
    p.fused_slab = ( p.leaf_cull && !c.reach_cull ) ? 1u : 0u;
    if ( s->leaf_box_test && r.d_blob && terra_leaf_boxes_fit ( p, ( uint32_t ) s->leaf_boxes.size() ) ) {
        p.leaf_boxes = ( const DevLeafBox* ) ( ( const char* ) r.d_blob + s->blob.sec[kSecLeafBoxes].offset ); p.n_leaf_boxes = ( uint32_t ) s->leaf_boxes.size();
    }
    p.leaf_pairs = 0;
    if ( s->leaf_pair_form && r.d_blob && !s->leaf_pairs.empty() && p.lds_mode == 1 && p.leaf_rank ) p.leaf_pairs = ( uint32_t ) ( s->blob.sec[kSecLeafPairs].offset - s->blob.sec[kSecTris].offset );
    if ( p.leaf_pairs && ! ( p.leaf_pairs & 3u ) && p.n_leaf_boxes && s->leaf_nearest_first && s->pair_per_box ) p.leaf_pairs |= TERRA_LEAF_PAIRS_NEAREST;
    if ( p.lds_mode != 1 ) p.scene.sincos24 = nullptr;
    s->last_azimuth_table.store ( p.scene.sincos24 ? 1 : 0, std::memory_order_relaxed );
    s->last_call.store ( p.lds_mode == 2 ? ( r.dev.reach ? kTerraAmdCallFastTreeReach : kTerraAmdCallFastTree ) : ( p.leaf_cull ? kTerraAmdCallLeafCull : kTerraAmdCallReplica ), std::memory_order_relaxed );
    p.bsdf_kinds = s->bsdf_kinds;
    p.sampler_mode = 0; p.sampler_strata = ( uint32_t ) s->opts.strata;
    if ( s->sampler_integration && s->opts.sampling_method == kTerraSamplingMethodHalton ) p.sampler_mode = 1;
    if ( s->sampler_integration && s->opts.sampling_method == kTerraSamplingMethodStratified && s->opts.strata > 0 ) p.sampler_mode = 2;
    if ( p.sampler_mode ) p.bsdf_kinds |= TERRA_KIND_SAMPLER;
    if ( r.dev.env_nx && ( p.integrator == kTerraIntegratorDirect || p.integrator == kTerraIntegratorDirectMis ) ) p.bsdf_kinds |= TERRA_KIND_SAMPLER;
    else { p.scene.env_nx = 0; p.scene.env_ny = 0; }
    if ( s->env_mis && p.scene.env_nx && p.scene.env_monotone && p.integrator == kTerraIntegratorDirectMis ) p.bsdf_kinds |= TERRA_KIND_ENV_MIS;
    p.count_level = s->work_counters ? 2 : 0;
    return 0;
}

static uint64_t shard_pixels ( const DevRenderParams& p ) {
    uint64_t n = 0;
    const uint32_t tx = ( p.w + p.tile_size - 1 ) / p.tile_size, ty = ( p.h + p.tile_size - 1 ) / p.tile_size;
    for ( uint32_t t = p.rank; t < tx * ty; t += p.world ) {
        uint32_t x0 = ( t % tx ) * p.tile_size, y0 = ( t / tx ) * p.tile_size;
        n += ( uint64_t ) std::min ( p.tile_size, p.w - x0 ) * std::min ( p.tile_size, p.h - y0 );
    }
    return n;
}
static void account_launch ( Scene* s, const DevRenderParams& p ) {
    uint64_t px = shard_pixels ( p );
// ... 1461 lines not shown
extern "C" int terra_amd_unit_bsdf ( int kind, int n, float* surfaces47, const float* e3, const float* wo3, float* wi3, float* pdf, float* f3 ) {
    if ( need_device() ) return kTerraAmdErrNoDevice;
    if ( kind < kDevBsdfDiffuse || kind > kDevBsdfGlass ) return fail ( kTerraAmdErrBadArgument, "unknown bsdf kind %d", kind );
    Unit u; auto sf = u.inout ( surfaces47, 47 * ( size_t ) n ); auto e = u.in ( e3, 3 * ( size_t ) n ); auto wo = u.in ( wo3, 3 * ( size_t ) n );
    auto wi = u.out ( wi3, 3 * ( size_t ) n ); auto pd = u.out ( pdf, n ); auto f = u.out ( f3, 3 * ( size_t ) n );
    return u.finish ( u.ok ? terra_unit_bsdf ( kind, n, sf, e, wo, wi, pd, f ) : hipSuccess );
}
extern "C" int terra_amd_unit_bsdf_at ( int kind, int n, const float* surfaces47, const float* wi3, const float* wo3, float* pdf, float* f3 ) {
    if ( need_device() ) return kTerraAmdErrNoDevice;
    if ( kind < kDevBsdfDiffuse || kind > kDevBsdfGlass ) return fail ( kTerraAmdErrBadArgument, "unknown bsdf kind %d", kind );
    if ( n <= 0 || !surfaces47 || !wi3 || !wo3 || !pdf || !f3 ) return fail ( kTerraAmdErrBadArgument, "terra_amd_unit_bsdf_at: null array or no items" );
    Unit u; auto sf = u.in ( surfaces47, 47 * ( size_t ) n ); auto wi = u.in ( wi3, 3 * ( size_t ) n ); auto wo = u.in ( wo3, 3 * ( size_t ) n );
    auto pd = u.out ( pdf, n ); auto f = u.out ( f3, 3 * ( size_t ) n );
    return u.finish ( u.ok ? terra_unit_bsdf_at ( kind, n, sf, wi, wo, pd, f ) : hipSuccess );
}
extern "C" int terra_amd_unit_camera ( const TerraCamera* cam, size_t fb_w, size_t fb_h, int n, const uint32_t* xy2, float jitter, const float* r2, float* dirs3 ) {
    if ( need_device() ) return kTerraAmdErrNoDevice;
    DevRenderParams p; memset ( &p, 0, sizeof p );
    fill_camera ( cam, fb_w, fb_h, p );
    p.jitter = jitter; p.fb_w = ( uint32_t ) fb_w; p.fb_h = ( uint32_t ) fb_h;
    Unit u; auto a = u.in ( xy2, 2 * ( size_t ) n ); auto b = u.in ( r2, 2 * ( size_t ) n ); auto o = u.out ( dirs3, 3 * ( size_t ) n );
    return u.finish ( u.ok ? terra_unit_camera ( p, n, a, b, o ) : hipSuccess );
}
extern "C" int terra_amd_unit_lens_rays ( const TerraCamera* cam, const TerraAmdLens* lens, size_t fb_w, size_t fb_h, int n, const uint32_t* xy2, float jitter, const float* r4, TerraAmdRay* out_rays ) {
    DevLens L;
    if ( int rc = fill_lens ( cam, lens, "terra_amd_unit_lens_rays", L ) ) return rc;
    if ( n < 0 || fb_w == 0 || fb_h == 0 || ( n && ( !xy2 || !r4 || !out_rays ) ) ) return fail ( kTerraAmdErrBadArgument, "terra_amd_unit_lens_rays: null array or empty frame" );
    if ( need_device() ) return kTerraAmdErrNoDevice;
    DevRenderParams p; memset ( &p, 0, sizeof p );
    fill_camera ( cam, fb_w, fb_h, p );
    p.jitter = jitter; p.fb_w = ( uint32_t ) fb_w; p.fb_h = ( uint32_t ) fb_h;
    Unit u; auto a = u.in ( xy2, 2 * ( size_t ) n ); auto b = u.in ( r4, 4 * ( size_t ) n ); auto o = u.out ( reinterpret_cast<float*> ( out_rays ), 8 * ( size_t ) n );
    return u.finish ( u.ok ? terra_unit_lens_rays ( p, L, n, a, b, o ) : hipSuccess );
}
extern "C" int terra_amd_unit_point_rays ( const TerraAmdPointSampling* ps, int n, const TerraAmdPoint* points, const float* g2, TerraAmdRay* out_rays ) {
    DevPointSampling D;
    if ( int rc = fill_point_sampling ( ps, "terra_amd_unit_point_rays", D ) ) return rc;
    if ( n < 0 || ( n && ( !points || !g2 || !out_rays ) ) ) return fail ( kTerraAmdErrBadArgument, "terra_amd_unit_point_rays: null array or negative count" );
    if ( need_device() ) return kTerraAmdErrNoDevice;
    Unit u; auto a = u.in ( reinterpret_cast<const float*> ( points ), 8 * ( size_t ) n ); auto b = u.in ( g2, 2 * ( size_t ) n ); auto o = u.out ( reinterpret_cast<float*> ( out_rays ), 8 * ( size_t ) n );
    return u.finish ( u.ok ? terra_unit_point_rays ( D, n, a, b, o ) : hipSuccess );
}
extern "C" int terra_amd_unit_tonemap ( int op, float gamma, int n, float* colors3 ) {
    if ( need_device() ) return kTerraAmdErrNoDevice;
    Unit u; auto c = u.inout ( colors3, 3 * ( size_t ) n );
    return u.finish ( u.ok ? terra_unit_tonemap ( op, gamma, n, c ) : hipSuccess );
}
extern "C" int terra_amd_unit_math ( int fn, int n, const float* x, const float* y, float* out ) {
    if ( need_device() ) return kTerraAmdErrNoDevice;
    Unit u; auto a = u.in ( x, n ); auto b = u.in ( y ? y : x, n ); auto o = u.out ( out, n );
    return u.finish ( u.ok ? terra_unit_math ( fn, n, a, b, o ) : hipSuccess );
}
extern "C" int terra_amd_unit_exact_div ( int op, const float* a, const float* b, const float* c, uint64_t first, uint64_t count, float denominator, float reciprocal, uint64_t seed,
                                           uint32_t* helper_bits, uint32_t* plain_bits, uint64_t* mismatches, uint32_t* first_bad ) {
    if ( need_device() ) return kTerraAmdErrNoDevice;
    if ( op < 0 || op > 4 || !mismatches || !first_bad ) return fail ( kTerraAmdErrBadArgument, "exact_div unit: op %d, or no place for the mismatch count and records", op );
    const bool explicit_set = a != nullptr;
    if ( explicit_set && ( op == 3 || !helper_bits || !plain_bits || ( ( op == 2 || op == 4 ) && !b ) || ( op == 4 && !c ) || count > ( 1ull << 28 ) ) )
        return fail ( kTerraAmdErrBadArgument, "exact_div unit: the explicit form of op %d needs its input and output arrays (op 3 has none), at most 2^28 elements", op );
    const size_t n = explicit_set ? ( size_t ) count : 0, per = op == 4 ? 3 : 1;
    Unit u;
    const float* da = explicit_set ? u.in ( a, n ) : nullptr; const float* db = explicit_set && ( op == 2 || op == 4 ) ? u.in ( b, n ) : nullptr; const float* dc = explicit_set && op == 4 ? u.in ( c, n ) : nullptr;
    uint32_t* dh = explicit_set ? u.out ( helper_bits, per * n ) : nullptr; uint32_t* dp = explicit_set ? u.out ( plain_bits, per * n ) : nullptr;
    *mismatches = 0;
    unsigned long long* dm = reinterpret_cast<unsigned long long*> ( u.inout ( mismatches, 1 ) ); uint32_t* dr = u.out ( first_bad, 9 * 16 );
    return u.finish ( u.ok ? terra_unit_exact_div ( op, da, db, dc, first, count, denominator, reciprocal, seed, dh, dp, dm, dr ) : hipSuccess );
}
extern "C" int terra_amd_unit_exact_sqrt ( int op, const float* a, const float* b, const float* c, uint64_t first, uint64_t count, uint64_t seed,
                                            uint32_t* helper_bits, uint32_t* plain_bits, uint64_t* mismatches, uint32_t* first_bad ) {
    if ( need_device() ) return kTerraAmdErrNoDevice;
    if ( op < 0 || op > 4 || !mismatches || !first_bad ) return fail ( kTerraAmdErrBadArgument, "exact_sqrt unit: op %d, or no place for the mismatch count and records", op );
    const bool explicit_set = a != nullptr, three = op == 2 || op == 4;
    if ( explicit_set && ( !helper_bits || !plain_bits || ( three && ( !b || !c ) ) || count > ( 1ull << 26 ) ) )
        return fail ( kTerraAmdErrBadArgument, "exact_sqrt unit: the explicit form of op %d needs its input and output arrays, at most 2^26 elements", op );
    const size_t n = explicit_set ? ( size_t ) count : 0, per = op == 2 ? 9 : ( op == 4 ? 3 : 1 );
    Unit u;
    const float* da = explicit_set ? u.in ( a, n ) : nullptr; const float* db = explicit_set && three ? u.in ( b, n ) : nullptr; const float* dc = explicit_set && three ? u.in ( c, n ) : nullptr;
    uint32_t* dh = explicit_set ? u.out ( helper_bits, per * n ) : nullptr; uint32_t* dp = explicit_set ? u.out ( plain_bits, per * n ) : nullptr;
    *mismatches = 0;
    unsigned long long* dm = reinterpret_cast<unsigned long long*> ( u.inout ( mismatches, 1 ) ); uint32_t* dr = u.out ( first_bad, 21 * 16 );
    return u.finish ( u.ok ? terra_unit_exact_sqrt ( op, da, db, dc, first, count, seed, dh, dp, dm, dr ) : hipSuccess );
}

extern "C" int terra_amd_unit_half_outward ( const double* x, int n, int up, uint16_t* out ) {
    if ( n < 0 || ( n && ( !x || !out ) ) ) return fail ( kTerraAmdErrBadArgument, "null array" );
    for ( int i = 0; i < n; ++i ) out[i] = fastbvh::half_outward ( x[i], up != 0 );
    return 0;
}

extern "C" int terra_amd_unit_stratified ( const uint32_t* seeds, int nseeds, int strata, int samples_per_stratum, int n, float* out2 ) {
    if ( need_device() ) return kTerraAmdErrNoDevice;
    if ( nseeds < 0 || n < 0 || strata < 1 || samples_per_stratum < 1 ) return fail ( kTerraAmdErrBadArgument, "stratified sampler: strata and samples per stratum must be positive" );
    if ( ( long long ) n > ( long long ) strata * strata * samples_per_stratum ) return fail ( kTerraAmdErrBadArgument, "stratified sampler: %d pairs requested but strata^2 * samples = %lld (the reference asserts, src/Terra.c:716)", n, ( long long ) strata * strata * samples_per_stratum );
    Unit u; auto ds = u.in ( seeds, nseeds ); auto o = u.out ( out2, ( size_t ) nseeds * n * 2 );
    return u.finish ( u.ok ? terra_unit_stratified ( ds, nseeds, strata, samples_per_stratum, n, o ) : hipSuccess );
}
extern "C" int terra_amd_unit_halton ( int first, int n, float* out2 ) {
    if ( need_device() ) return kTerraAmdErrNoDevice;
    if ( first < 0 || n < 0 ) return fail ( kTerraAmdErrBadArgument, "halton: negative index" );
    Unit u; auto o = u.out ( out2, ( size_t ) n * 2 );
    return u.finish ( u.ok ? terra_unit_halton ( first, n, o ) : hipSuccess );
}
extern "C" int terra_amd_unit_distribution_1d ( const float* f, size_t n, const float* e, int m, float* x, float* pdf, uint32_t* idx, float* cdf_out, float* integral_out ) {
    if ( need_device() ) return kTerraAmdErrNoDevice;
    if ( n == 0 || n > 0x7fffffffu || m < 0 ) return fail ( kTerraAmdErrBadArgument, "distribution: empty table" );
    std::vector<float> cdf_tmp ( cdf_out ? 0 : n ); float integral_tmp = 0.f; uint32_t mono = 0;
    Unit u; auto df = u.in ( f, n ); auto de = u.in ( e, ( size_t ) m );
    auto dc = u.out ( cdf_out ? cdf_out : cdf_tmp.data(), n ); auto di = u.out ( integral_out ? integral_out : &integral_tmp, 1 ); auto dm = u.out ( &mono, 1 );
    auto dx = u.out ( x, ( size_t ) m ); auto dp = u.out ( pdf, ( size_t ) m ); auto dk = u.out ( idx, ( size_t ) m );
    return u.finish ( u.ok ? terra_unit_distribution_1d ( df, ( uint32_t ) n, dc, di, dm, de, m, dx, dp, dk ) : hipSuccess );
}
extern "C" int terra_amd_unit_distribution_2d ( const float* f, size_t nx, size_t ny, const float* e12, int m, float* xy2, float* pdf, float* marginal_cdf_out ) {
    if ( need_device() ) return kTerraAmdErrNoDevice;
    if ( nx == 0 || ny == 0 || nx * ny > 0x7fffffffu || m < 0 ) return fail ( kTerraAmdErrBadArgument, "distribution: empty table" );
    std::vector<float> cdf ( nx * ny ), integrals ( ny + 1 ), mcdf_tmp ( marginal_cdf_out ? 0 : ny ); std::vector<uint32_t> mono ( ny + 1 );
    Unit u; auto df = u.in ( f, nx * ny ); auto de = u.in ( e12, ( size_t ) m * 2 );
    auto dc = u.out ( cdf.data(), nx * ny ); auto di = u.out ( integrals.data(), ny + 1 ); auto dmc = u.out ( marginal_cdf_out ? marginal_cdf_out : mcdf_tmp.data(), ny ); auto dm = u.out ( mono.data(), ny + 1 );
    auto dxy = u.out ( xy2, ( size_t ) m * 2 ); auto dp = u.out ( pdf, ( size_t ) m );
    return u.finish ( u.ok ? terra_unit_distribution_2d ( df, ( uint32_t ) nx, ( uint32_t ) ny, dc, di, dmc, dm, de, m, dxy, dp ) : hipSuccess );
}
extern "C" int terra_amd_unit_distribution_2d_pdf ( const float* f, size_t nx, size_t ny, const float* xy2, int m, float* pdf ) {
    if ( need_device() ) return kTerraAmdErrNoDevice;
    if ( nx == 0 || ny == 0 || nx * ny > 0x7fffffffu || m < 0 ) return fail ( kTerraAmdErrBadArgument, "distribution: empty table" );
    std::vector<float> cdf ( nx * ny ), integrals ( ny + 1 ), mcdf ( ny ); std::vector<uint32_t> mono ( ny + 1 );
    Unit u; auto df = u.in ( f, nx * ny ); auto dxy = u.in ( xy2, ( size_t ) m * 2 );
    auto dc = u.out ( cdf.data(), nx * ny ); auto di = u.out ( integrals.data(), ny + 1 ); auto dmc = u.out ( mcdf.data(), ny ); auto dm = u.out ( mono.data(), ny + 1 );
    auto dp = u.out ( pdf, ( size_t ) m );
    return u.finish ( u.ok ? terra_unit_distribution_2d_pdf ( df, ( uint32_t ) nx, ( uint32_t ) ny, dc, di, dmc, dm, dxy, m, dp ) : hipSuccess );
}

extern "C" int terra_amd_unit_azimuth24 ( uint32_t* mismatches ) {
    if ( need_device() ) return kTerraAmdErrNoDevice;
    if ( !mismatches ) return fail ( kTerraAmdErrBadArgument, "unit azimuth: null count" );
    float2* table = nullptr; float2* computed = nullptr; uint32_t* count = nullptr;
    hipError_t e = hipMalloc ( ( void** ) &table, sizeof ( float2 ) << 24 );
    if ( e == hipSuccess ) e = hipMalloc ( ( void** ) &computed, sizeof ( float2 ) << 24 );
    if ( e == hipSuccess ) e = hipMalloc ( ( void** ) &count, sizeof ( uint32_t ) );
    if ( e == hipSuccess ) e = hipMemset ( count, 0, sizeof ( uint32_t ) );
    if ( e == hipSuccess ) e = terra_fill_sincos24 ( table, nullptr );
    if ( e == hipSuccess ) e = terra_unit_azimuth24 ( table, computed, count );
    if ( e == hipSuccess ) e = hipDeviceSynchronize();
    if ( e == hipSuccess ) e = hipMemcpy ( mismatches, count, sizeof ( uint32_t ), hipMemcpyDeviceToHost );
    ( void ) hipFree ( table ); ( void ) hipFree ( computed ); ( void ) hipFree ( count );
    if ( e != hipSuccess ) { ( void ) hipGetLastError(); return fail ( kTerraAmdErrLaunch, "unit azimuth: %s", hipGetErrorString ( e ) ); }
    return 0;
}

static int unit_texture ( const TerraTexture* t, int n, const float* in, int in_width, float* out3, hipError_t ( *launch ) ( const DevTexture*, int, const float*, float* ) ) {
    if ( need_device() ) return kTerraAmdErrNoDevice;
    if ( !t || !texture_ok ( t ) || n < 0 || ( n && ( !in || !out3 ) ) ) return fail ( kTerraAmdErrBadArgument, "unit texture lookup: invalid texture or null array" );
    BlobLayout L { std::vector<Section> ( kSecTextures + 1 ), std::vector<DevTexture> ( 1 ) };
    layout_textures ( L, { t } );
    void* d_blob = nullptr;
    int rc = new_blob ( L, &d_blob );
    if ( !rc ) {
        Unit u; auto a = u.in ( in, ( size_t ) in_width * n ); auto o = u.out ( out3, 3 * ( size_t ) n );
        rc = u.finish ( u.ok ? launch ( ( const DevTexture* ) ( ( char* ) d_blob + L.sec[kSecTexDesc].offset ), n, a, o ) : hipSuccess );
    }
    ( void ) hipFree ( d_blob );
    return rc;
}
extern "C" int terra_amd_unit_texture_sample ( const TerraTexture* t, int n, const float* uv2, float* out3 ) { return unit_texture ( t, n, uv2, 2, out3, terra_unit_texture_sample ); }
extern "C" int terra_amd_unit_texture_latlong ( const TerraTexture* t, int n, const float* dir3, float* out3 ) { return unit_texture ( t, n, dir3, 3, out3, terra_unit_texture_latlong ); }
```

terra_amd/csrc/shading_device.h:

```cpp
#pragma once
#include "traverse_fast.h"

TD float texture_coord ( float u ) { return u > -1.f ? fminf ( u, 4294967040.f ) : 0.f; }
TD V3 texture_read ( const DevTexture& t, uint32_t x, uint32_t y ) {
    const uint32_t W = t.width, H = t.height;
    if ( t.address_mode == 2 ) { x = x < W - 1 ? x : W - 1; y = y < H - 1 ? y : H - 1; }
    else if ( t.address_mode == 0 ) { x %= W; y %= H; }
    else if ( ( x / W ) % 2 == 0 ) { x %= W; y %= H; }
    else { x = W - ( x % W ); y = H - ( y % H ); x = x < W - 1 ? x : W - 1; y = y < H - 1 ? y : H - 1; }
    const size_t e = ( ( size_t ) y * W + x ) * t.components;
    if ( t.depth == 1 ) {
        const uint8_t* p = reinterpret_cast<const uint8_t*> ( t.data ) + e;
        return v3 ( p[0] / 255.f, p[1] / 255.f, p[2] / 255.f );
    }
    const float* p = reinterpret_cast<const float*> ( t.data ) + e;
    return v3 ( p[0], p[1], p[2] );
}
TD V3 texture_sample ( const DevTexture& t, float u, float v ) {
    u = texture_coord ( u ); v = texture_coord ( v );
    uint32_t ix = ( uint32_t ) u, iy = ( uint32_t ) v;
    if ( t.filter == 0 ) return texture_read ( t, ix, iy );
    if ( t.filter != 1 ) return v3 ( 0, 0, 0 );
    uint32_t x2 = ix + 1 < t.width - 1 ? ix + 1 : t.width - 1, y2 = iy + 1 < t.height - 1 ? iy + 1 : t.height - 1;
    V3 n1 = texture_read ( t, ix, iy ), n2 = texture_read ( t, x2, iy ), n3 = texture_read ( t, ix, y2 ), n4 = texture_read ( t, x2, y2 );
    float wu = u - ( float ) ix, wv = v - ( float ) iy, wou = 1.f - wu, wov = 1.f - wv;
    return v3 ( ( n1.x * wou + n2.x * wu ) * wov + ( n3.x * wou + n4.x * wu ) * wv,
                ( n1.y * wou + n2.y * wu ) * wov + ( n3.y * wou + n4.y * wu ) * wv,
                ( n1.z * wou + n2.z * wu ) * wov + ( n3.z * wou + n4.z * wu ) * wv );
}

#define TERRA_PI_F 3.1416926535f
#define TERRA_INV_PI_F 0x1.45f06p-2f
static_assert ( TERRA_INV_PI_F == 1.f / TERRA_PI_F, "the literal is the compiler's own correctly rounded quotient" );
TD V3 environment_eval ( const DevScene& sc, V3 dir ) {
    if ( sc.env_mode == 1 ) return v3 ( sc.env_color[0], sc.env_color[1], sc.env_color[2] );
    const DevTexture& t = sc.textures[sc.env_tex];
    V3 d = normalize ( dir );
    float theta = tdm_acosf ( d.y );
    float phi = tdm_atan2f ( d.z, d.x ) + TERRA_PI_F;
    uint32_t u = ( uint32_t ) texture_coord ( ( phi / ( 2 * TERRA_PI_F ) ) * ( float ) t.width );
    uint32_t v = ( uint32_t ) texture_coord ( ( theta / TERRA_PI_F ) * ( float ) t.height );
    return texture_read ( t, u, v );
}

struct Surface {
    V3    normal;
    V3    emissive;
    V3    attr[4];
    float ior;
    int   bsdf;
};

template <int MODE, int KINDS>
TD void surface_init ( const Tracer& T, uint32_t ti, V3 point, Surface& sf, uint32_t& object_out, uint32_t& tri_in_object_out, uint32_t& nattr_out ) {
    float4 t0, t1, t2, p0, p1, p2, p3x;
    if ( MODE == 1 ) {
        const float4* lt = reinterpret_cast<const float4*> ( T.l_tris );
        t0 = lt[3 * ti]; t1 = lt[3 * ti + 1]; t2 = lt[3 * ti + 2];
        p0 = T.l_props[4 * ti]; p1 = T.l_props[4 * ti + 1]; p2 = T.l_props[4 * ti + 2]; p3x = T.l_props[4 * ti + 3];
    } else {
        const float4* tris = reinterpret_cast<const float4*> ( MODE >= 2 ? T.sc.fast_tris : T.sc.tris );
        const float4* props = reinterpret_cast<const float4*> ( T.sc.props );
        t0 = tris[3 * ti]; t1 = tris[3 * ti + 1]; t2 = tris[3 * ti + 2];
        uint32_t pi = ti;
        if ( MODE >= 2 ) pi = T.sc.mats[__float_as_uint ( t0.w )].first_tri + __float_as_uint ( t1.w );
        p0 = props[4 * pi]; p1 = props[4 * pi + 1]; p2 = props[4 * pi + 2]; p3x = props[4 * pi + 3];
    }
    uint32_t object = __float_as_uint ( t0.w );
    object_out = object; tri_in_object_out = __float_as_uint ( t1.w );
    float u, v;
    if ( MODE == 1 && T.l_consts ) {
        const float4 c0 = T.l_consts[3 * ti], c1 = T.l_consts[3 * ti + 1], c2 = T.l_consts[3 * ti + 2];
        const V3 e0 = v3 ( c0.x, c0.y, c0.z ), e1 = v3 ( c0.w, c1.x, c1.y ), p = point - v3 ( t0.x, t0.y, t0.z );
        const float d00 = c1.z, d11 = c1.w, d01 = c2.x, div = c2.y;
        const float dp0 = dot ( p, e0 ), dp1 = dot ( p, e1 );
        const float nu = d11 * dp0 - d01 * dp1, nv = d00 * dp1 - d01 * dp0;
        if ( ( int ) __float_as_uint ( c2.w ) & xd_in_range ( nu ) & xd_in_range ( nv ) ) { u = xd_div_short ( nu, div, c2.z ); v = xd_div_short ( nv, div, c2.z ); }
        else { u = nu / div; v = nv / div; }
    } else {
        V3 ta, tb, tc; tri_vertices ( t0, t1, t2, ta, tb, tc );
        V3 e0 = tb - ta, e1 = tc - ta, p = point - ta;
        float d00 = dot ( e0, e0 ), d11 = dot ( e1, e1 ), d01 = dot ( e0, e1 );
        float dp0 = dot ( p, e0 ), dp1 = dot ( p, e1 );
        float div = d00 * d11 - d01 * d01;
        div2_exact ( d11 * dp0 - d01 * dp1, d00 * dp1 - d01 * dp0, div, u, v );
    }
    float w = 1 - u - v;
    V3 na = v3 ( p0.x, p0.y, p0.z ), nb = v3 ( p0.w, p1.x, p1.y ), nc = v3 ( p1.z, p1.w, p2.x );
    sf.normal = normalize ( ( nc * v + nb * u ) + na * w );
    const DevMaterial& m = T.l_mats[object];
    sf.emissive = v3p ( m.emissive );
    #pragma unroll
    for ( int i = 0; i < 4; ++i ) sf.attr[i] = v3p ( m.attributes[i] );
    if ( ( KINDS & TERRA_KIND_TEX ) && m.any_texture ) {
        V3 pa2 = v3 ( p2.y, p2.z, 0.f );
        V3 pb2 = v3 ( p2.w, p3x.x, 0.f );
        V3 pc2 = v3 ( p3x.y, p3x.z, 0.f );
        float tx = ( pc2.x * v + pb2.x * u ) + pa2.x * w;
        float ty = ( pc2.y * v + pb2.y * u ) + pa2.y * w;
        #pragma unroll
        for ( int i = 0; i < 4; ++i ) if ( m.tex[i] >= 0 ) sf.attr[i] = texture_sample ( T.sc.textures[m.tex[i]], tx, ty );
        if ( m.tex[TERRA_DEV_MAX_ATTR] >= 0 ) sf.emissive = texture_sample ( T.sc.textures[m.tex[TERRA_DEV_MAX_ATTR]], tx, ty );
    }
    sf.bsdf = m.bsdf;
    sf.ior = m.ior;
    nattr_out = m.attributes_count;
}

struct RaycastResult { bool hit; uint32_t object, tri_in_object, tri; V3 point; };

struct Azimuth { float sn, cs; uint32_t k; int kind; };
struct PathDraws { float e0, e1, e2, e3; Azimuth az; };
template <int MODE> TD const float2* azimuth_table ( const DevScene& sc ) { return MODE == 1 ? sc.sincos24 : nullptr; }
template <int COUNT> TD PathDraws path_draw ( const float2* sincos24, Pcg32& rb, Counters& c );

template <int COUNT, int MODE, int KINDS>
TD RaycastResult scene_raycast ( const Tracer& T, const Ray& in, Surface& sf, Counters& c, PathDraws* pre = nullptr, Pcg32* rb = nullptr, bool guarded = false ) {
    Ray r = in;
    r.o = r.o + r.d * 0.001f;
    constexpr bool MASKS = ray_start_masks_for ( COUNT, MODE, KINDS );
    if ( COUNT ) ++c.rays;
    Closest best;
    if constexpr ( MASKS ) { V3 o_perm; const RayStateMasks st = ray_start_masks ( r, o_perm ); best = bvh_traverse_from<COUNT, MODE> ( T, r, st, o_perm, c, __all ( guarded ) != 0 ); }
    else {
    RayState st = ray_state_init ( r );
    if ( MODE >= 2 ) { ClosestRanked b2 = bvh_traverse_fast<COUNT, MODE == 3> ( T, r, st, c ); best.depth = b2.depth; best.tri = b2.tri; }
    else best = bvh_traverse<COUNT, MODE> ( T, r, st, c );
    }
    RaycastResult res; res.hit = best.tri != 0xffffffffu; res.tri = best.tri; res.object = 0; res.tri_in_object = 0;
    res.point = res.hit ? r.o + r.d * best.depth : v3 ( FLT_MAX, FLT_MAX, FLT_MAX );
    if ( res.hit ) {
        uint32_t nattr;
        if ( pre ) *pre = path_draw<COUNT> ( azimuth_table<MODE> ( T.sc ), *rb, c );
        surface_init<MODE, KINDS> ( T, best.tri, res.point, sf, res.object, res.tri_in_object, nattr );
        if ( MODE >= 2 ) res.tri = T.sc.mats[res.object].first_tri + res.tri_in_object;
        if ( COUNT ) ++c.hits;
        if ( COUNT == 2 ) c.attr_fetches += nattr + 1;
    }
    return res;
}

template <int COUNT, int MODE, bool MASKS = false>
TD uint32_t scene_raycast_triangle ( const Tracer& T, const Ray& in, Counters& c, uint32_t expected ) {
    Ray r = in;
    r.o = r.o + r.d * 0.001f;
    V3 o_masks = v3 ( 0, 0, 0 );
    const auto st = [&] { if constexpr ( MASKS ) return ray_start_masks ( r, o_masks ); else return ray_state_init ( r ); } ();
    if ( COUNT ) ++c.rays;
    if constexpr ( MODE == 2 && COUNT == 0 ) {
        const V3 o_perm = permuted ( r.o, st );
        ClosestRanked best;
        if ( !fast_expect ( T, st, o_perm, expected, best ) ) return 0xffffffffu;
        int* top = T.stack; uint32_t hand = TERRA_FAST_ROOT_IN_HAND, held = 0u;
        traverse_fast_resume<COUNT> ( T, r, st, o_perm, best, top, hand, held, 0, c, false, true );
        return best.tri == TERRA_TRI_EXPECTED ? expected : 0xffffffffu;
    }
    if constexpr ( MODE == 1 && COUNT == 0 ) {
        const V3 o_perm = MASKS ? o_masks : permuted ( r.o, st );
        float depth;
        if ( !watertight_permuted ( tri_perm_lds ( T.l_tris + 12 * expected, st ), o_perm, st, depth ) ) return 0xffffffffu;
        Closest best; best.depth = __uint_as_float ( __float_as_uint ( depth + 0.f ) + 1u ); best.tri = 0xffffffffu;
        if ( T.pairs ) { best.depth = depth; best.tri = terra_pair_key ( __float_as_uint ( T.l_tris[12 * expected + 11] ), expected ); }
        if ( T.fused && __all ( ray_is_tame ( r ) ) ) traverse_loops<COUNT, MODE, true, true, true> ( T, r, st, o_perm, best, c, expected );
        else if ( __all ( ray_is_regular ( r ) ) ) traverse_loops<COUNT, MODE, true, false, true> ( T, r, st, o_perm, best, c, expected );
        else traverse_loops<COUNT, MODE, false, false, true> ( T, r, st, o_perm, best, c, expected );
        if ( T.pairs ) return best.tri != 0u ? expected : 0xffffffffu;
        return best.tri;
    }
    uint32_t tri;
    if ( MODE >= 2 ) { const ClosestRanked b2 = bvh_traverse_fast<COUNT, MODE == 3> ( T, r, st, c ); tri = b2.tri; }
    else tri = bvh_traverse<COUNT, MODE> ( T, r, st, c ).tri;
    if ( tri == 0xffffffffu ) return tri;
    uint32_t object;
    if ( MODE == 1 ) object = __float_as_uint ( T.l_tris[12 * tri + 3] );
    else {
        const float4* tris = reinterpret_cast<const float4*> ( MODE >= 2 ? T.sc.fast_tris : T.sc.tris );
        const float4 t0 = tris[3 * tri];
        object = __float_as_uint ( t0.w );
        if ( MODE >= 2 ) tri = T.sc.mats[object].first_tri + __float_as_uint ( tris[3 * tri + 1].w );
    }
    if ( COUNT ) ++c.hits;
    if ( COUNT == 2 ) c.attr_fetches += T.l_mats[object].attributes_count + 1;
    return tri;
}

TD V3 surface_origin ( const Surface& sf, V3 p ) { return p + sf.normal * 0.0001f; }
TD Ray surface_ray ( const Surface& sf, V3 p, V3 d ) { return make_ray ( surface_origin ( sf, p ), d ); }


static_assert ( TDM_AZIMUTH_SCALE == 2 * TERRA_PI_F, "tdm_azimuth24's scale is the samplers' 2 * terra_PI" );
TD Azimuth azimuth_none() { Azimuth a; a.sn = 0.f; a.cs = 1.f; a.k = 0u; a.kind = 0; return a; }
TD Azimuth azimuth_fetch_index ( const float2* tab, uint32_t k ) {
    Azimuth a = azimuth_none();
    if ( tab ) { const float2 v = tab[k]; a.cs = v.x; a.sn = v.y; a.kind = 1; }
    else { a.k = k; a.kind = 2; }
    return a;
}
TD Azimuth azimuth_fetch ( const float2* tab, float e ) {
    const float x = e * 16777216.f;
    if ( e >= 0.f && x < 16777216.f ) {
        const uint32_t k = ( uint32_t ) x;
        if ( ( float ) k == x ) return azimuth_fetch_index ( tab, k );
    }
    return azimuth_none();
}
TD void azimuth_sincos ( const Azimuth& az, float e, float& sn, float& cs ) {
    if ( az.kind == 1 ) { sn = az.sn; cs = az.cs; }
    else if ( az.kind == 2 ) tdm_azimuth24 ( az.k, sn, cs );
    else tdm_sincosf_pair ( 2 * TERRA_PI_F * e, sn, cs );
}

TD V3 diffuse_sample ( const Surface& sf, float e1, float e2, const Azimuth& az ) {
    float r = sqrt_exact ( e1 );
    float sn, cs;
    azimuth_sincos ( az, e2, sn, cs );
    float x = r * cs;
    float z = r * sn;
// ... 150 lines not shown
```

terra_amd/csrc/trace_geometry.h:

```cpp
#pragma once
#include "trace_math.h"

TD void camera_film ( const DevRenderParams& p, uint32_t px, uint32_t py, float r1, float r2, float& sx, float& sy ) {
    float dx = -p.jitter + 2 * r1 * p.jitter;
    float dy = -p.jitter + 2 * r2 * p.jitter;
    float ndc_x, ndc_y; div2_exact_rk ( ( float ) px + 0.5f + dx, ( float ) py + 0.5f + dy, ( float ) p.fb_w, p.inv_fb_w, ( float ) p.fb_h, p.inv_fb_h, ndc_x, ndc_y );
    sx = 2 * ndc_x - 1;
    sy = 1 - 2 * ndc_y;
}
TD V3 camera_rotate ( const DevRenderParams& p, V3 d ) {
    return v3 ( p.cam_rot[0] * d.x + p.cam_rot[1] * d.y + p.cam_rot[2] * d.z,
                p.cam_rot[3] * d.x + p.cam_rot[4] * d.y + p.cam_rot[5] * d.z,
                p.cam_rot[6] * d.x + p.cam_rot[7] * d.y + p.cam_rot[8] * d.z );
}
TD V3 camera_sample ( const DevRenderParams& p, uint32_t px, uint32_t py, float r1, float r2 ) {
    float sx, sy; camera_film ( p, px, py, r1, r2, sx, sy );
    float fx = sx * p.aspect * p.tan_half_fov;
    float fy = sy * p.tan_half_fov;
    V3 d = normalize ( v3 ( fx, fy, 1.f ) );
    return camera_rotate ( p, d );
}

TD void concentric_disk ( float l1, float l2, float& u, float& v ) {
    const float kPi2 = tdm_float ( 0x3FC90FDBu ), kPi4 = tdm_float ( 0x3F490FDBu );
    const float a = 2 * l1 - 1, b = 2 * l2 - 1;
    u = 0.f; v = 0.f;
    if ( ! ( a == 0.f && b == 0.f ) ) {
        float r, phi;
        if ( fabsf ( a ) > fabsf ( b ) ) { r = a; phi = kPi4 * ( b / a ); }
        else { r = b; phi = kPi2 - kPi4 * ( a / b ); }
        float sp, cp; tdm_sincosf_pair ( phi, sp, cp );
        u = r * cp; v = r * sp;
    }
}

TD bool lens_draws ( const DevLens& L ) { return L.model == 0 && L.lens_radius > 0.f; }
TD void lens_sample ( const DevRenderParams& p, const DevLens& L, uint32_t px, uint32_t py, float r1, float r2, float l1, float l2, V3& ro, V3& rd ) {
    const float kPi = tdm_float ( 0x40490FDBu ), kPi2 = tdm_float ( 0x3FC90FDBu );
    float sx, sy; camera_film ( p, px, py, r1, r2, sx, sy );
    const V3 pos = v3 ( p.cam_pos[0], p.cam_pos[1], p.cam_pos[2] );
    float Lx = 0.f, Ly = 0.f;
    bool shifted = false;
    if ( L.model == 0 ) {
        const float fx = sx * p.aspect * p.tan_half_fov;
        const float fy = sy * p.tan_half_fov;
        const V3 d = normalize ( v3 ( fx, fy, 1.f ) );
        if ( L.lens_radius > 0.f ) {
            float u, v; concentric_disk ( l1, l2, u, v );
            Lx = L.lens_radius * u; Ly = L.lens_radius * v; shifted = true;
            const float t = L.focus_distance / d.z;
            const V3 F = v3 ( d.x * t, d.y * t, d.z * t );
            rd = camera_rotate ( p, normalize ( v3 ( F.x - Lx, F.y - Ly, F.z ) ) );
        } else rd = camera_rotate ( p, d );
    } else if ( L.model == 1 ) {
        Lx = ( sx * p.aspect ) * L.ortho_half; Ly = sy * L.ortho_half; shifted = true;
        rd = camera_rotate ( p, v3 ( 0.f, 0.f, 1.f ) );
    } else if ( L.model == 2 ) {
        const float phi = sx * kPi, theta = sy * kPi2;
        float st, ct, sp, cp; tdm_sincosf_pair ( theta, st, ct ); tdm_sincosf_pair ( phi, sp, cp );
        rd = camera_rotate ( p, v3 ( ct * sp, st, ct * cp ) );
    } else {
        const float ux = sx * p.aspect, uy = sy, rr = sqrtf ( ux * ux + uy * uy ), theta = rr * L.fisheye_half;
        if ( rr == 0.f ) rd = camera_rotate ( p, v3 ( 0.f, 0.f, 1.f ) );
        else { float st, ct; tdm_sincosf_pair ( theta, st, ct ); rd = camera_rotate ( p, v3 ( ( st * ux ) / rr, ( st * uy ) / rr, ct ) ); }
    }
    ro = shifted ? v3 ( pos.x + ( p.cam_rot[0] * Lx + p.cam_rot[1] * Ly ), pos.y + ( p.cam_rot[3] * Lx + p.cam_rot[4] * Ly ), pos.z + ( p.cam_rot[6] * Lx + p.cam_rot[7] * Ly ) ) : pos;
}

TD bool point_inactive ( V3 pos, V3 nrm ) {
    const bool finite = fabsf ( pos.x ) < INFINITY && fabsf ( pos.y ) < INFINITY && fabsf ( pos.z ) < INFINITY && fabsf ( nrm.x ) < INFINITY && fabsf ( nrm.y ) < INFINITY && fabsf ( nrm.z ) < INFINITY;
    const float q = nrm.x * nrm.x + nrm.y * nrm.y + nrm.z * nrm.z;
    return !finite || ! ( q > 0.f && q < INFINITY );
}
TD void point_sample ( const DevPointSampling& S, V3 pos, V3 nrm, float g1, float g2, V3& ro, V3& rd ) {
    const V3 n = normalize ( nrm );
    const float s = copysignf ( 1.f, n.z );
    const float a = -1.f / ( s + n.z );
    const float b = ( n.x * n.y ) * a;
    const V3 t = v3 ( 1.f + ( s * ( n.x * n.x ) ) * a, s * b, ( -s ) * n.x );
    const V3 bt = v3 ( b, s + ( n.y * n.y ) * a, -n.y );
    float x, y, z;
    if ( S.distribution == 0 ) {
        concentric_disk ( g1, g2, x, y );
        z = sqrtf ( fmaxf ( 0.f, ( 1.f - x * x ) - y * y ) );
    } else {
        z = 1.f - 2 * g1;
        const float r = sqrtf ( fmaxf ( 0.f, 1.f - z * z ) );
        const float phi = tdm_float ( 0x40C90FDBu ) * g2;
        float sp, cp; tdm_sincosf_pair ( phi, sp, cp );
        x = r * cp; y = r * sp;
    }
    rd = normalize ( v3 ( ( x * t.x + y * bt.x ) + z * n.x, ( x * t.y + y * bt.y ) + z * n.y, ( x * t.z + y * bt.z ) + z * n.z ) );
    ro = pos;
}

TD bool ray_aabb ( const Ray& r, V3 bmin, V3 bmax, float* tmin_out, float* tmax_out ) {
    float t1 = ( bmin.x - r.o.x ) * r.inv.x;
    float t2 = ( bmax.x - r.o.x ) * r.inv.x;
    float tmin = sel_min ( t1, t2 ), tmax = sel_max ( t1, t2 );
    t1 = ( bmin.y - r.o.y ) * r.inv.y;
    t2 = ( bmax.y - r.o.y ) * r.inv.y;
    tmin = sel_max ( tmin, sel_min ( t1, t2 ) ); tmax = sel_min ( tmax, sel_max ( t1, t2 ) );
    t1 = ( bmin.z - r.o.z ) * r.inv.z;
// ... 10 lines not shown
    float t1x = ( bmin.x - r.o.x ) * r.inv.x, t2x = ( bmax.x - r.o.x ) * r.inv.x;
    float t1y = ( bmin.y - r.o.y ) * r.inv.y, t2y = ( bmax.y - r.o.y ) * r.inv.y;
    float t1z = ( bmin.z - r.o.z ) * r.inv.z, t2z = ( bmax.z - r.o.z ) * r.inv.z;
    if ( FAST ) {
        float tmin = __builtin_fmaxf ( __builtin_fmaxf ( __builtin_fminf ( t1x, t2x ), __builtin_fminf ( t1y, t2y ) ), __builtin_fminf ( t1z, t2z ) );
        float tmax = __builtin_fminf ( __builtin_fminf ( __builtin_fmaxf ( t1x, t2x ), __builtin_fmaxf ( t1y, t2y ) ), __builtin_fmaxf ( t1z, t2z ) );
        return tmax > __builtin_fmaxf ( tmin, 0.f );
    }
    float tmin = sel_min ( t1x, t2x ), tmax = sel_max ( t1x, t2x );
    tmin = sel_max ( tmin, sel_min ( t1y, t2y ) ); tmax = sel_min ( tmax, sel_max ( t1y, t2y ) );
    tmin = sel_max ( tmin, sel_min ( t1z, t2z ) ); tmax = sel_min ( tmax, sel_max ( t1z, t2z ) );
    return tmax > sel_max ( tmin, 0.f );
}

TD bool ray_is_regular ( const Ray& r ) {
    uint32_t ax = tdm_bits ( r.inv.x ) & 0x7fffffffu, ay = tdm_bits ( r.inv.y ) & 0x7fffffffu, az = tdm_bits ( r.inv.z ) & 0x7fffffffu;
    return ax - 1u < 0x7f7fffffu && ay - 1u < 0x7f7fffffu && az - 1u < 0x7f7fffffu;
}

TD bool ray_is_tame ( const Ray& r ) {
    uint32_t ax = tdm_bits ( r.inv.x ) & 0x7fffffffu, ay = tdm_bits ( r.inv.y ) & 0x7fffffffu, az = tdm_bits ( r.inv.z ) & 0x7fffffffu;
    return ax - 1u < 0x6f7fffffu && ay - 1u < 0x6f7fffffu && az - 1u < 0x6f7fffffu;
}
TD bool slab_near_far ( float nx, float fx, float ny, float fy, float nz, float fz, const Ray& r ) {
    float tnx = ( nx - r.o.x ) * r.inv.x, tfx = ( fx - r.o.x ) * r.inv.x;
    float tny = ( ny - r.o.y ) * r.inv.y, tfy = ( fy - r.o.y ) * r.inv.y;
    float tnz = ( nz - r.o.z ) * r.inv.z, tfz = ( fz - r.o.z ) * r.inv.z;
    float tmin = __builtin_fmaxf ( __builtin_fmaxf ( tnx, tny ), tnz );
    float tmax = __builtin_fminf ( __builtin_fminf ( tfx, tfy ), tfz );
    return tmax > __builtin_fmaxf ( tmin, 0.f );
}

TD bool slab_near_far_fused ( float nx, float fx, float ny, float fy, float nz, float fz, const Ray& r, V3 oi, float& t_enter ) {
    float tnx = __builtin_fmaf ( nx, r.inv.x, -oi.x ), tfx = __builtin_fmaf ( fx, r.inv.x, -oi.x );
    float tny = __builtin_fmaf ( ny, r.inv.y, -oi.y ), tfy = __builtin_fmaf ( fy, r.inv.y, -oi.y );
    float tnz = __builtin_fmaf ( nz, r.inv.z, -oi.z ), tfz = __builtin_fmaf ( fz, r.inv.z, -oi.z );
    float tmin = __builtin_fmaxf ( __builtin_fmaxf ( tnx, tny ), tnz );
    float tmax = __builtin_fminf ( __builtin_fminf ( tfx, tfy ), tfz );
    t_enter = __builtin_fmaxf ( tmin, 0.f );
    return tmax > t_enter;
}

TD RayState ray_state_init ( const Ray& r ) {
    float ax = fabsf ( r.d.x ), ay = fabsf ( r.d.y ), az = fabsf ( r.d.z );
    int iz = ax > ay ? ( ax > az ? 0 : 2 ) : ( ay > az ? 1 : 2 );
    int ix = iz + 1 == 3 ? 0 : iz + 1;
    int iy = ix + 1 == 3 ? 0 : ix + 1;
    if ( pick ( r.d, iz ) < 0.f ) { int t = ix; ix = iy; iy = t; }
    RayState s;
    s.scalez = pick ( r.inv, iz );
    s.shearx = pick ( r.d, ix ) * s.scalez;
    s.sheary = pick ( r.d, iy ) * s.scalez;
    s.ix = ix; s.iy = iy; s.iz = iz;
    return s;
}

TD RayStateMasks ray_start_masks ( const Ray& r, V3& o_perm ) {
    const float ax = fabsf ( r.d.x ), ay = fabsf ( r.d.y ), az = fabsf ( r.d.z );
    const bool xy = ax > ay, xz = ax > az, yz = ay > az;
    const bool z0 = xy & xz, z1 = !xy & yz;
    const auto at_z = [&] ( V3 a ) { return z0 ? a.x : ( z1 ? a.y : a.z ); };
    const bool flip = at_z ( r.d ) < 0.f;
    const auto at_xy = [&] ( V3 a, float& px, float& py ) {
        const float u = z0 ? a.y : ( z1 ? a.z : a.x ), v = z0 ? a.z : ( z1 ? a.x : a.y );
        px = flip ? v : u; py = flip ? u : v;
    };
    RayStateMasks s;
    s.perm = ( z0 ? 0u : ( z1 ? 2u : 4u ) ) + ( flip ? 1u : 0u );
    asm volatile ( "" : "+v" ( s.perm ) );
    s.ix = ( int ) ( ( 0x429u >> ( 2u * s.perm ) ) & 3u ); s.iy = ( int ) ( ( 0x186u >> ( 2u * s.perm ) ) & 3u ); s.iz = ( int ) ( s.perm >> 1 );
    s.scalez = at_z ( r.inv );
    float dix, diy; at_xy ( r.d, dix, diy );
    s.shearx = dix * s.scalez;
    s.sheary = diy * s.scalez;
    at_xy ( r.o, o_perm.x, o_perm.y ); o_perm.z = at_z ( r.o );
    return s;
}
#if TERRA_RAY_SOURCE
#define TERRA_RAY_START_CAMERA 0
#else
#define TERRA_RAY_START_CAMERA 1
#endif
TD constexpr bool ray_start_masks_for ( int COUNT, int MODE, int KINDS ) { return TERRA_RAY_START_CAMERA && MODE == 1 && COUNT == 0 && KINDS == 1; }

TD void tri_vertices ( float4 t0, float4 t1, float4 t2, V3& a, V3& b, V3& c ) { a = v3 ( t0.x, t0.y, t0.z ); b = v3 ( t1.x, t1.y, t1.z ); c = v3 ( t2.x, t2.y, t2.z ); }
TD void tri_vertices ( const float4* tris, uint32_t i, V3& a, V3& b, V3& c ) { tri_vertices ( tris[3 * i], tris[3 * i + 1], tris[3 * i + 2], a, b, c ); }

struct TriPerm { float a[3], b[3], c[3]; };
TD TriPerm tri_perm_lds ( const float* t, const RayState& s ) {
    TriPerm p;
    p.a[0] = t[s.ix]; p.a[1] = t[s.iy]; p.a[2] = t[s.iz];
    p.b[0] = t[4 + s.ix]; p.b[1] = t[4 + s.iy]; p.b[2] = t[4 + s.iz];
    p.c[0] = t[8 + s.ix]; p.c[1] = t[8 + s.iy]; p.c[2] = t[8 + s.iz];
    return p;
}
TD TriPerm tri_perm ( float4 t0, float4 t1, float4 t2, const RayState& s ) {
    const V3 va = v3 ( t0.x, t0.y, t0.z ), vb = v3 ( t1.x, t1.y, t1.z ), vc = v3 ( t2.x, t2.y, t2.z );
    TriPerm p;
    p.a[0] = pick ( va, s.ix ); p.a[1] = pick ( va, s.iy ); p.a[2] = pick ( va, s.iz );
    p.b[0] = pick ( vb, s.ix ); p.b[1] = pick ( vb, s.iy ); p.b[2] = pick ( vb, s.iz );
    p.c[0] = pick ( vc, s.ix ); p.c[1] = pick ( vc, s.iy ); p.c[2] = pick ( vc, s.iz );
    return p;
}

struct TriHit { float u, v, w, depth; V3 point; };

TD bool watertight ( const Ray& r, const RayState& s, V3 ta, V3 tb, V3 tc, TriHit& h ) {
    V3 A = ta - r.o, B = tb - r.o, C = tc - r.o;
    float Aiz = pick ( A, s.iz ), Biz = pick ( B, s.iz ), Ciz = pick ( C, s.iz );
    float Ax = pick ( A, s.ix ) - s.shearx * Aiz, Ay = pick ( A, s.iy ) - s.sheary * Aiz;
    float Bx = pick ( B, s.ix ) - s.shearx * Biz, By = pick ( B, s.iy ) - s.sheary * Biz;
    float Cx = pick ( C, s.ix ) - s.shearx * Ciz, Cy = pick ( C, s.iy ) - s.sheary * Ciz;
    float U = Cx * By - Cy * Bx;
    float V = Ax * Cy - Ay * Cx;
    float W = Bx * Ay - By * Ax;
    if ( U == 0.f || V == 0.f || W == 0.f ) {
        U = ( float ) ( ( double ) Cx * ( double ) By - ( double ) Cy * ( double ) Bx );
        V = ( float ) ( ( double ) Ax * ( double ) Cy - ( double ) Ay * ( double ) Cx );
        W = ( float ) ( ( double ) Bx * ( double ) Ay - ( double ) By * ( double ) Ax );
    }
    uint32_t sign = tdm_bits ( U ) & 0x80000000u;
    if ( ( ( tdm_bits ( V ) ^ tdm_bits ( U ) ) | ( tdm_bits ( W ) ^ tdm_bits ( U ) ) ) & 0x80000000u ) return false;
    float det = U + V + W;
    if ( det == 0.f ) return false;
    float Az = s.scalez * Aiz, Bz = s.scalez * Biz, Cz = s.scalez * Ciz;
    float depth = U * Az + V * Bz + W * Cz;
    if ( tdm_float ( tdm_bits ( depth ) ^ sign ) < 0.f ) return false;
    float inv_det = 1.f / det;
    h.u = U * inv_det; h.v = V * inv_det; h.w = W * inv_det;
    h.depth = depth * inv_det;
    h.point = r.o + r.d * h.depth;
    return true;
}

TD bool watertight_permuted ( const TriPerm& t, V3 o, const RayState& s, float& depth_out ) {
    float Aix = t.a[0] - o.x, Aiy = t.a[1] - o.y, Aiz = t.a[2] - o.z;
    float Bix = t.b[0] - o.x, Biy = t.b[1] - o.y, Biz = t.b[2] - o.z;
    float Cix = t.c[0] - o.x, Ciy = t.c[1] - o.y, Ciz = t.c[2] - o.z;
    float Ax = Aix - s.shearx * Aiz, Ay = Aiy - s.sheary * Aiz;
    float Bx = Bix - s.shearx * Biz, By = Biy - s.sheary * Biz;
    float Cx = Cix - s.shearx * Ciz, Cy = Ciy - s.sheary * Ciz;
    float U = Cx * By - Cy * Bx;
    float V = Ax * Cy - Ay * Cx;
    float W = Bx * Ay - By * Ax;
    if ( U == 0.f || V == 0.f || W == 0.f ) {
        U = ( float ) ( ( double ) Cx * ( double ) By - ( double ) Cy * ( double ) Bx );
        V = ( float ) ( ( double ) Ax * ( double ) Cy - ( double ) Ay * ( double ) Cx );
        W = ( float ) ( ( double ) Bx * ( double ) Ay - ( double ) By * ( double ) Ax );
    }
    uint32_t sign = tdm_bits ( U ) & 0x80000000u;
    if ( ( ( tdm_bits ( V ) ^ tdm_bits ( U ) ) | ( tdm_bits ( W ) ^ tdm_bits ( U ) ) ) & 0x80000000u ) return false;
    float det = U + V + W;
    if ( det == 0.f ) return false;
    float Az = s.scalez * Aiz, Bz = s.scalez * Biz, Cz = s.scalez * Ciz;
    float depth = U * Az + V * Bz + W * Cz;
    if ( tdm_float ( tdm_bits ( depth ) ^ sign ) < 0.f ) return false;
    float inv_det = 1.f / det;
    depth_out = depth * inv_det;
    return true;
}

struct PairPerm { float p0[3], p1[3], p2[3], p3[3]; };
TD bool pair_finish ( float U, float V, float W, float Aiz, float Biz, float Ciz, const RayState& s, float& depth_out ) {
    uint32_t sign = tdm_bits ( U ) & 0x80000000u;
    float det = U + V + W;
    if ( det == 0.f ) return false;
// ... 70 lines not shown
```

terra_amd/csrc/trace_math.h:

```cpp
#pragma once
#include <hip/hip_runtime.h>
#include <float.h>
#include "dev_types.h"
#include "dev_math.h"
#include "rng.h"
#include "sampling_device.h"
#include "exact_div.h"
#include "exact_sqrt.h"

#define TD __device__ __forceinline__

struct V3 { float x, y, z; };

TD V3 v3 ( float x, float y, float z ) { V3 r; r.x = x; r.y = y; r.z = z; return r; }
TD V3 v3p ( const float* p ) { return v3 ( p[0], p[1], p[2] ); }
TD V3 operator+ ( V3 a, V3 b ) { return v3 ( a.x + b.x, a.y + b.y, a.z + b.z ); }
TD V3 operator- ( V3 a, V3 b ) { return v3 ( a.x - b.x, a.y - b.y, a.z - b.z ); }
TD V3 operator* ( V3 a, float s ) { return v3 ( a.x * s, a.y * s, a.z * s ); }
TD V3 had ( V3 a, V3 b ) { return v3 ( a.x * b.x, a.y * b.y, a.z * b.z ); }
TD V3 neg ( V3 a ) { return v3 ( -a.x, -a.y, -a.z ); }
TD float dot ( V3 a, V3 b ) { return a.x * b.x + a.y * b.y + a.z * b.z; }
TD V3 cross ( V3 a, V3 b ) { return v3 ( a.y * b.z - a.z * b.y, a.z * b.x - a.x * b.z, a.x * b.y - a.y * b.x ); }
TD float length2 ( V3 a ) { return a.x * a.x + a.y * a.y + a.z * a.z; }
TD float length ( V3 a ) { return sqrtf ( length2 ( a ) ); }
TD V3 normalize_plain ( V3 a ) { float l = sqrtf ( length2 ( a ) ); return v3 ( a.x / l, a.y / l, a.z / l ); }
TD V3 normalize ( V3 a ) { float l = sqrt_exact ( length2 ( a ) ); V3 r; xd_normalize3 ( a.x, a.y, a.z, l, r.x, r.y, r.z ); return r; }
TD float sel_min ( float a, float b ) { return a < b ? a : b; }
TD float sel_max ( float a, float b ) { return a > b ? a : b; }
TD float pick ( V3 a, int i ) { return i == 0 ? a.x : ( i == 1 ? a.y : a.z ); }

struct Basis { float r0[3], r1[3], r2[3]; };
TD V3 basis_apply ( const Basis& m, V3 v ) {
    return v3 ( m.r0[0] * v.x + m.r0[1] * v.y + m.r0[2] * v.z,
                m.r1[0] * v.x + m.r1[1] * v.y + m.r1[2] * v.z,
                m.r2[0] * v.x + m.r2[1] * v.y + m.r2[2] * v.z );
}
TD Basis basis_of ( V3 t, V3 n ) {
    V3 b = cross ( n, t );
    Basis m;
    m.r0[0] = t.x; m.r0[1] = n.x; m.r0[2] = b.x;
    m.r1[0] = t.y; m.r1[1] = n.y; m.r1[2] = b.y;
    m.r2[0] = t.z; m.r2[1] = n.z; m.r2[2] = b.z;
    return m;
}
TD Basis make_basis_plain ( V3 n ) {
    V3 t;
    if ( fabsf ( n.x ) > fabsf ( n.y ) ) {
        float k = sqrtf ( n.x * n.x + n.z * n.z );
        t = v3 ( n.z * k, 0.f * k, -n.x * k );
    } else {
        float k = sqrtf ( n.y * n.y + n.z * n.z );
        t = v3 ( 0.f * k, -n.z * k, n.y * k );
    }
    return basis_of ( t, n );
}
TD Basis make_basis ( V3 n ) {
    const bool c = fabsf ( n.x ) > fabsf ( n.y );
    const float a = c ? n.x : n.y;
    const float k = sqrt_exact ( a * a + n.z * n.z );
    return basis_of ( v3 ( ( c ? n.z : 0.f ) * k, ( c ? 0.f : -n.z ) * k, ( c ? -n.x : n.y ) * k ), n );
}

struct Ray { V3 o, d, inv; };
TD Ray make_ray ( V3 o, V3 d ) { Ray r; r.o = o; r.d = d; rcp3_exact ( d.x, d.y, d.z, r.inv.x, r.inv.y, r.inv.z ); return r; }
TD Ray make_ray_guarded ( V3 o, V3 d, bool& guarded ) {
    Ray r; r.o = o; r.d = d;
    guarded = ( xd_rcp_ok ( d.x ) & xd_rcp_ok ( d.y ) & xd_rcp_ok ( d.z ) ) != 0;
    if ( guarded ) { r.inv.x = xd_rcp_short ( d.x ); r.inv.y = xd_rcp_short ( d.y ); r.inv.z = xd_rcp_short ( d.z ); }
    else { r.inv.x = 1.f / d.x; r.inv.y = 1.f / d.y; r.inv.z = 1.f / d.z; }
    return r;
}

struct RayState { float shearx, sheary, scalez; int ix, iy, iz; };
TD V3 permuted ( V3 a, const RayState& s ) { return v3 ( pick ( a, s.ix ), pick ( a, s.iy ), pick ( a, s.iz ) ); }
TD uint32_t ray_perm ( const RayState& s ) { return 2u * ( uint32_t ) s.iz + ( uint32_t ) ( s.ix != ( s.iz == 2 ? 0 : s.iz + 1 ) ); }
struct RayStateMasks : RayState { uint32_t perm; };
TD uint32_t ray_perm ( const RayStateMasks& s ) { return s.perm; }
```

terra_amd/csrc/unit_kernels.hip:

```cpp
#include <hip/hip_runtime.h>
#include "trace_device.h"
#include "sampling_device.h"
#include "kernels.h"

#define UNIT_GRID(n) dim3 ( ( ( n ) + 255 ) / 256 ), dim3 ( 256 )

__global__ void k_pcg ( const uint32_t* seeds, int nseeds, int n, float* out ) {
    int i = blockIdx.x * blockDim.x + threadIdx.x;
    if ( i >= nseeds ) return;
    Pcg32 a; a.state = 0; a.inc = 1;
    trng_next ( a ); a.state += seeds[i]; trng_next ( a );
    for ( int j = 0; j < n; ++j ) out[ ( size_t ) i * n + j] = trng_a_float ( a );
}
hipError_t terra_unit_pcg ( const uint32_t* seeds, int nseeds, int n, float* out ) {
    hipLaunchKernelGGL ( k_pcg, UNIT_GRID ( nseeds ), 0, 0, seeds, nseeds, n, out );
    return hipGetLastError();
}

__global__ void k_stream_keys ( uint64_t seed, const uint64_t* pix, const uint64_t* k, int n, uint64_t* out3 ) {
    int i = blockIdx.x * blockDim.x + threadIdx.x;
    if ( i >= n ) return;
    PixelStreams s = trng_pixel_streams ( seed, pix[i], k[i] );
    out3[3 * i] = s.seedA; out3[3 * i + 1] = s.b.state; out3[3 * i + 2] = s.b.inc;
}
// ... 431 lines not shown
    float a, b; halton_pair ( first + i, a, b );
    out2[2 * i] = a; out2[2 * i + 1] = b;
}
hipError_t terra_unit_halton ( int first, int n, float* out2 ) {
    hipLaunchKernelGGL ( k_halton, UNIT_GRID ( n ), 0, 0, first, n, out2 );
    return hipGetLastError();
}
__global__ void k_dist_rows ( const float* f, uint32_t nx, uint32_t ny, float* cdf, float* integrals, uint32_t* monotone ) {
    uint32_t r = blockIdx.x * blockDim.x + threadIdx.x;
    if ( r >= ny ) return;
    integrals[r] = distribution_row_init ( f + ( size_t ) nx * r, nx, cdf + ( size_t ) nx * r, monotone + r );
}
__global__ void k_dist_marginal ( uint32_t ny, float* integrals, float* mcdf, uint32_t* monotone ) {
    if ( blockIdx.x || threadIdx.x ) return;
    integrals[ny] = distribution_row_init ( integrals, ny, mcdf, monotone + ny );
}
__global__ void k_dist_sample_1d ( const float* f, const float* cdf, uint32_t n, const float* integral, const uint32_t* monotone, const float* e, int m, float* x, float* pdf, uint32_t* idx ) {
    int i = blockIdx.x * blockDim.x + threadIdx.x;
    if ( i >= m ) return;
    DevDistribution1D d = { f, cdf, n, integral[0], monotone[0] };
    float p = 0.f; uint32_t k = 0;
    x[i] = distribution_sample ( d, e[i], &p, &k );
    pdf[i] = p; idx[i] = k;
}
__global__ void k_dist_sample_2d ( const float* f, const float* cdf, uint32_t nx, uint32_t ny, const float* integrals, const float* mcdf, const uint32_t* monotone, const float* e12, int m, float* xy2, float* pdf ) {
    int i = blockIdx.x * blockDim.x + threadIdx.x;
    if ( i >= m ) return;
    DevDistribution1D marginal = { integrals, mcdf, ny, integrals[ny], monotone[ny] };
    float p0 = 0.f, p1 = 0.f; uint32_t row = 0;
    const float s1 = distribution_sample ( marginal, e12[2 * i], &p0, &row );
    if ( s1 == FLT_MAX ) { xy2[2 * i] = xy2[2 * i + 1] = FLT_MAX; pdf[i] = 0.f; return; }
    DevDistribution1D cond = { f + ( size_t ) nx * row, cdf + ( size_t ) nx * row, nx, integrals[row], monotone[row] };
    const float s2 = distribution_sample ( cond, e12[2 * i + 1], &p1, nullptr );
    xy2[2 * i] = s1; xy2[2 * i + 1] = s2; pdf[i] = p0 * p1;
}
hipError_t terra_unit_distribution_1d ( const float* f, uint32_t n, float* cdf, float* integral, uint32_t* monotone, const float* e, int m, float* x, float* pdf, uint32_t* idx ) {
    hipLaunchKernelGGL ( k_dist_rows, dim3 ( 1 ), dim3 ( 64 ), 0, 0, f, n, 1u, cdf, integral, monotone );
    if ( m > 0 ) hipLaunchKernelGGL ( k_dist_sample_1d, UNIT_GRID ( m ), 0, 0, f, cdf, n, integral, monotone, e, m, x, pdf, idx );
    return hipGetLastError();
}
hipError_t terra_unit_distribution_2d ( const float* f, uint32_t nx, uint32_t ny, float* cdf, float* integrals, float* mcdf, uint32_t* monotone, const float* e12, int m, float* xy2, float* pdf ) {
    hipLaunchKernelGGL ( k_dist_rows, UNIT_GRID ( ny ), 0, 0, f, nx, ny, cdf, integrals, monotone );
    hipLaunchKernelGGL ( k_dist_marginal, dim3 ( 1 ), dim3 ( 64 ), 0, 0, ny, integrals, mcdf, monotone );
    if ( m > 0 ) hipLaunchKernelGGL ( k_dist_sample_2d, UNIT_GRID ( m ), 0, 0, f, cdf, nx, ny, integrals, mcdf, monotone, e12, m, xy2, pdf );
    return hipGetLastError();
}
__global__ void k_dist_pdf_2d ( const float* f, uint32_t nx, uint32_t ny, const float* integrals, const float* xy2, int m, float* pdf ) {
    int i = blockIdx.x * blockDim.x + threadIdx.x;
    if ( i >= m ) return;
    const float v = xy2[2 * i], u = xy2[2 * i + 1];
    uint32_t row = v > 0.f ? ( uint32_t ) ( v * ( float ) ny ) : 0u, col = u > 0.f ? ( uint32_t ) ( u * ( float ) nx ) : 0u;
    row = row < ny - 1u ? row : ny - 1u; col = col < nx - 1u ? col : nx - 1u;
    pdf[i] = distribution_2d_prob ( f, integrals, nx, integrals[ny], row, col );
}
hipError_t terra_unit_distribution_2d_pdf ( const float* f, uint32_t nx, uint32_t ny, float* cdf, float* integrals, float* mcdf, uint32_t* monotone, const float* xy2, int m, float* pdf ) {
    hipLaunchKernelGGL ( k_dist_rows, UNIT_GRID ( ny ), 0, 0, f, nx, ny, cdf, integrals, monotone );
    hipLaunchKernelGGL ( k_dist_marginal, dim3 ( 1 ), dim3 ( 64 ), 0, 0, ny, integrals, mcdf, monotone );
    if ( m > 0 ) hipLaunchKernelGGL ( k_dist_pdf_2d, UNIT_GRID ( m ), 0, 0, f, nx, ny, integrals, xy2, m, pdf );
    return hipGetLastError();
}

__global__ __launch_bounds__ ( 256 ) void terra_sincos24_kernel ( float2* table ) {
    const uint32_t k = blockIdx.x * 256u + threadIdx.x;
    float sn, cs;
    tdm_sincosf_pair ( 2 * TERRA_PI_F * ( ( float ) k * 0x1p-24f ), sn, cs );
    table[k] = make_float2 ( cs, sn );
}
hipError_t terra_fill_sincos24 ( float2* table, hipStream_t stream ) {
    hipLaunchKernelGGL ( terra_sincos24_kernel, dim3 ( ( 1u << 24 ) / 256u ), dim3 ( 256 ), 0, stream, table );
    return hipGetLastError();
}
__global__ __launch_bounds__ ( 256 ) void k_azimuth24 ( const float2* table, float2* computed, uint32_t* mismatches ) {
    const uint32_t k = blockIdx.x * 256u + threadIdx.x;
    float sn, cs;
    tdm_azimuth24 ( k, sn, cs );
    computed[k] = make_float2 ( cs, sn );
    const float2 t = table[k];
    if ( __float_as_uint ( t.x ) != __float_as_uint ( cs ) || __float_as_uint ( t.y ) != __float_as_uint ( sn ) ) atomicAdd ( mismatches, 1u );
}
hipError_t terra_unit_azimuth24 ( const float2* table, float2* computed, uint32_t* mismatches ) {
    hipLaunchKernelGGL ( k_azimuth24, dim3 ( ( 1u << 24 ) / 256u ), dim3 ( 256 ), 0, 0, table, computed, mismatches );
    return hipGetLastError();
}
```

Before: 37480 Msamples/s.

## Stage ray, surface and bounce math with wave-uniform guard fallback

Adds staged versions of ray setup, surface interpolation/normalization and diffuse path continuation. Each stage first runs the short reciprocal/sqrt sequences unconditionally, records whether every input was in the guarded range, and reruns the exact guarded path only if any lane in the wave failed. A host-computed camera-limits flag selects this when the camera parameters allow it. The aim is to drop per-lane divergent branches and slow division fallbacks in the hot shading loop. The cost is occasional double computation and more code and register pressure.

New measurement: 39250 Msamples/s, median of 6. +4.7%, better.

```diff
diff --git a/include/terra_amd.h b/include/terra_amd.h
--- a/include/terra_amd.h
+++ b/include/terra_amd.h
@@ -509,6 +509,8 @@
 int terra_amd_unit_distribution_2d ( const float* f, size_t nx, size_t ny, const float* e12, int m, float* xy2, float* pdf, float* marginal_cdf_out );
 int terra_amd_unit_distribution_2d_pdf ( const float* f, size_t nx, size_t ny, const float* xy2, int m, float* pdf );
 int terra_amd_unit_azimuth24 ( uint32_t* mismatches );
+int terra_amd_shade_stage_info ( const TerraCamera* cam, size_t fb_w, size_t fb_h, int* s1_guarded );
+int terra_amd_unit_shade_stages ( int stage, int drops, const float* rows, uint64_t count, uint32_t* staged, uint32_t* guarded, uint32_t* mask, uint32_t* full_mask, uint32_t* mismatches );
 int terra_amd_unit_texture_sample ( const TerraTexture* texture, int n, const float* uv2, float* out3 );
 int terra_amd_unit_texture_latlong ( const TerraTexture* texture, int n, const float* dir3, float* out3 );
 
diff --git a/terra_amd/csrc/dev_types.h b/terra_amd/csrc/dev_types.h
--- a/terra_amd/csrc/dev_types.h
+++ b/terra_amd/csrc/dev_types.h
@@ -210,12 +210,20 @@
     uint32_t fused_slab;
     uint32_t leaf_rank;
     uint32_t sampler_mode, sampler_strata;
+    uint32_t shade_s1_guarded;
     const uint32_t* job_live;
     const DevLeafBox* leaf_boxes;
     uint32_t n_leaf_boxes;
     uint32_t leaf_pairs;
     float    inv_fb_w, inv_fb_h;
 };
+static_assert ( sizeof ( DevRenderParams ) == 576 && offsetof ( DevRenderParams, job_live ) == 544, "shade_s1_guarded sits in padding: no field of the launch parameters moved" );
+inline bool terra_camera_stage_limits ( float aspect, float tan_half_fov, const float* rot9 ) {
+    const float at = aspect * tan_half_fov;
+    bool ok = at >= 0x1p-30f && at <= 0x1p20f && tan_half_fov >= 0x1p-30f && tan_half_fov <= 0x1p20f;
+    for ( int i = 0; i < 9; ++i ) ok = ok && ( rot9[i] >= -2.f && rot9[i] <= 2.f );
+    return ok;
+}
 struct DevLaunchMask { const uint32_t* words; uint32_t* live_blocks; };
 #define TERRA_CLASS_MASKED 3u
 struct DevRayRenderParams : DevRenderParams { const float4* rays; };
diff --git a/terra_amd/csrc/exact_div.h b/terra_amd/csrc/exact_div.h
--- a/terra_amd/csrc/exact_div.h
+++ b/terra_amd/csrc/exact_div.h
@@ -63,6 +63,15 @@
     qx = x / l; qy = y / l; qz = z / l;
 }
 
+XD int roulette_scale_ok ( float pr ) { return ( int ) ( pr >= 0.f ) & ( int ) ( pr <= 0x1p60f ); }
+XD float roulette_scale_short ( float pr ) {
+    const double d = ( double ) pr + 1e-4;
+    double y = __builtin_amdgcn_rcp ( d );
+    double e = __builtin_fma ( -d, y, 1.0 ); y = __builtin_fma ( y, e, y );
+    e = __builtin_fma ( -d, y, 1.0 ); y = __builtin_fma ( y, e, y );
+    e = __builtin_fma ( -d, y, 1.0 ); y = __builtin_fma ( e, y, y );
+    return ( float ) y;
+}
 XD float roulette_scale ( float pr ) {
     const double d = ( double ) pr + 1e-4;
     if ( ( int ) ( pr >= 0.f ) & ( int ) ( pr <= 0x1p60f ) ) {
@@ -74,3 +83,26 @@
     }
     return ( float ) ( 1.0 / d );
 }
+
+template <bool SHORT> XD float xd_site_rcp ( float d, int guard, int& ok ) {
+    if constexpr ( SHORT ) { ok &= guard; return xd_rcp_short ( d ); }
+    else { if ( guard ) return xd_rcp_short ( d ); return 1.f / d; }
+}
+template <bool SHORT> XD float xd_site_div_rk ( float x, float d, float r, int& ok ) {
+    if constexpr ( SHORT ) { ok &= xd_in_range ( x ); return xd_div_short ( x, d, r ); }
+    else return div_exact_rk ( x, d, r );
+}
+XD float xd_rcp_all_ones ( float d ) { return __uint_as_float ( ( 0x7e800000u - ( __float_as_uint ( d ) & 0x7f800000u ) ) | 1u | ( __float_as_uint ( d ) & 0x80000000u ) ); }
+XD float xd_rcp_short_any ( float d ) { return ( __float_as_uint ( d ) & 0x7fffffu ) == 0x7fffffu ? xd_rcp_all_ones ( d ) : xd_rcp_short ( d ); }
+XD int xd_normalize3_any_ok ( float x, float y, float z, float l ) {
+    return ( int ) ( l >= 0x1p-60f ) & ( int ) ( l <= 0x1p60f ) & xd_component_ok ( x ) & xd_component_ok ( y ) & xd_component_ok ( z );
+}
+template <bool SHORT> XD void xd_site_normalize3 ( float x, float y, float z, float l, float& qx, float& qy, float& qz, int& ok ) {
+    if constexpr ( SHORT ) {
+        ok &= xd_normalize3_any_ok ( x, y, z, l );
+        const float r = xd_rcp_short_any ( l );
+        qx = xd_div_short_pos ( x, l, r ); qy = xd_div_short_pos ( y, l, r ); qz = xd_div_short_pos ( z, l, r );
+    } else xd_normalize3 ( x, y, z, l, qx, qy, qz );
+}
+XD int xd_rcp_unit_ok ( float d ) { return ( int ) ( __builtin_fabsf ( d ) >= 0x1p-60f ) & ( int ) ( ( __float_as_uint ( d ) & 0x7fffffu ) != 0x7fffffu ); }
+XD int xd_rcp_clamped_ok ( float d ) { return ( int ) ( d <= 0x1p60f ) & ( int ) ( ( __float_as_uint ( d ) & 0x7fffffu ) != 0x7fffffu ); }
diff --git a/terra_amd/csrc/exact_sqrt.h b/terra_amd/csrc/exact_sqrt.h
--- a/terra_amd/csrc/exact_sqrt.h
+++ b/terra_amd/csrc/exact_sqrt.h
@@ -16,3 +16,8 @@
     if ( xs_in_range ( x ) ) return xs_sqrt_short ( x );
     return sqrtf ( x );
 }
+template <bool SHORT> XD float xs_site_sqrt ( float x, int guard, int& ok ) {
+    if constexpr ( SHORT ) { ok &= guard; return xs_sqrt_short ( x ); }
+    else { if ( guard ) return xs_sqrt_short ( x ); return sqrtf ( x ); }
+}
+XD int xs_variate_ok ( float e ) { return ( int ) ( e != 0.f ); }
diff --git a/terra_amd/csrc/integrators_device.h b/terra_amd/csrc/integrators_device.h
--- a/terra_amd/csrc/integrators_device.h
+++ b/terra_amd/csrc/integrators_device.h
@@ -342,6 +342,39 @@
     ++bounce;
     return bounce <= max_bounces;
 }
+template <bool SHORT, bool DROPS>
+TD int continue_stage ( V3 n, V3 albedo, V3 throughput, const PathDraws& d, V3& wi, V3& t, bool& go ) {
+    int ok = 1;
+    const float r = xs_site_sqrt<SHORT> ( d.e0, DROPS ? xs_variate_ok ( d.e0 ) : xs_in_range ( d.e0 ), ok );
+    float sn, cs;
+    azimuth_sincos ( d.az, d.e1, sn, cs );
+    const float x = r * cs, z = r * sn;
+    const float om = sel_max ( 0.f, 1 - d.e0 );
+    const float y = xs_site_sqrt<SHORT> ( om, DROPS ? 1 : xs_in_range ( om ), ok );
+    wi = normalize_site<SHORT> ( basis_apply ( make_basis_site<SHORT> ( n, ok ), v3 ( x, y, z ) ), ok );
+    const float pdf = sel_max ( xd_site_div_rk<SHORT> ( sel_max ( 0.f, dot ( n, wi ) ), TERRA_PI_F, TERRA_INV_PI_F, ok ), ( float ) 1e-4 );
+    const V3 f = ( albedo * ( float ) ( 1. / ( double ) TERRA_PI_F ) ) * xd_site_rcp<SHORT> ( pdf, DROPS ? xd_rcp_clamped_ok ( pdf ) : xd_rcp_ok ( pdf ), ok );
+    t = had ( throughput, f );
+    t = t * dot ( n, wi );
+    const float pr = sel_max ( t.x, sel_max ( t.y, t.z ) );
+    go = ! ( d.e3 > pr );
+    if constexpr ( SHORT ) {
+        ok &= roulette_scale_ok ( pr ) | ( int ) !go;
+        t = t * ( go ? roulette_scale_short ( pr ) : 1.f );
+    } else if ( go ) t = t * roulette_scale ( pr );
+    return ok;
+}
+TD bool path_continue_staged ( const Surface& sf, V3& throughput, uint32_t& bounce, uint32_t max_bounces, const PathDraws& d, V3& wi ) {
+    V3 t; bool go;
+    if constexpr ( TERRA_SHADE_STAGES != 0 ) {
+        if ( __any ( !continue_stage<true, TERRA_SHADE_DROPS != 0> ( sf.normal, sf.attr[0], throughput, d, wi, t, go ) ) )
+            continue_stage<false, false> ( sf.normal, sf.attr[0], throughput, d, wi, t, go );
+    } else continue_stage<false, TERRA_SHADE_DROPS != 0> ( sf.normal, sf.attr[0], throughput, d, wi, t, go );
+    throughput = t;
+    if ( !go ) return false;
+    ++bounce;
+    return bounce <= max_bounces;
+}
 struct SamplerPair { float u0, u1; bool on; };
 TD SamplerPair sampler_pair_none() { SamplerPair s; s.u0 = s.u1 = 0.f; s.on = false; return s; }
 TD void path_apply_sampler ( PathDraws& d, const SamplerPair& sp, uint32_t bounce ) {
diff --git a/terra_amd/csrc/kernels.h b/terra_amd/csrc/kernels.h
--- a/terra_amd/csrc/kernels.h
+++ b/terra_amd/csrc/kernels.h
@@ -85,6 +85,7 @@
 
 hipError_t terra_fill_sincos24 ( float2* table, hipStream_t stream );
 hipError_t terra_unit_azimuth24 ( const float2* table, float2* computed, uint32_t* mismatches );
+hipError_t terra_unit_shade_stages ( int stage, int drops, const float* rows, uint64_t n, uint32_t* staged, uint32_t* guarded, uint32_t* mask, uint32_t* full_mask, uint32_t* mismatches );
 
 hipError_t terra_unit_pcg ( const uint32_t* seeds, int nseeds, int n, float* out );
 hipError_t terra_unit_stream_keys ( uint64_t frame_seed, const uint64_t* pix, const uint64_t* k, int n, uint64_t* out3 );
diff --git a/terra_amd/csrc/render_kernels.hip b/terra_amd/csrc/render_kernels.hip
--- a/terra_amd/csrc/render_kernels.hip
+++ b/terra_amd/csrc/render_kernels.hip
@@ -428,7 +428,7 @@
 #define TERRA_JOB_NEXT() job_take<COUNT, MODE == 1> ( p, acc_lds, jb, rs, c, job_total, held )
 #else
 #define TERRA_LENS_RAY( ro, rd, r1, r2 )
-#define TERRA_PRIMARY_RAY( ro, rd, r1, r2 ) ro = cam_pos; rd = camera_sample ( p, jb.px, jb.py, r1, r2 )
+#define TERRA_PRIMARY_RAY( ro, rd, r1, r2 ) ro = cam_pos; rd = camera_direction<ray_start_masks_for ( COUNT, MODE, KINDS )> ( p, jb.px, jb.py, r1, r2 )
 #define TERRA_JOB_NEXT() job_next<COUNT, MODE == 1> ( p, acc_lds, jb, rs, c, job_total )
 #endif
 #if TERRA_RAY_SOURCE == 1 || TERRA_RAY_SOURCE == 3
@@ -652,7 +652,7 @@
         }
         if ( alive ) {
             bool guarded = false;
-            if constexpr ( ray_start_masks_for ( COUNT, MODE, KINDS ) ) ray = make_ray_guarded ( ro, rd, guarded ); else
+            if constexpr ( ray_start_masks_for ( COUNT, MODE, KINDS ) ) ray = make_ray_staged ( ro, rd, guarded, p.shade_s1_guarded ); else
             ray = make_ray ( ro, rd );
             Surface sf;
             PS_WAVE ( c, kPsRayIter ); PS_LANE ( c, kPsRayLanes );
@@ -663,11 +663,13 @@
             if ( h.hit ) {
                 PS_WAVE ( c, kPsShadeIter ); PS_LANE ( c, kPsShadeLanes );
                 V3 wo = neg ( ray.d ), wi;
+                constexpr bool STAGED = ray_start_masks_for ( COUNT, MODE, KINDS );
                 constexpr bool SPLIT_DIRECT = INTEGRATOR == 1 && ( KINDS & ( TERRA_KIND_TEX | TERRA_KIND_SAMPLER ) ) == 0;
                 if constexpr ( SPLIT_DIRECT ) {
                     Ray shadow_ray;
                     const DirectPending pend = direct_prepare<COUNT, KINDS, MODE> ( T, sf, h.point, wo, throughput, bounce, rs.b, c, shadow_ray );
                     pd = path_draw<COUNT> ( azimuth_table<MODE> ( T.sc ), rs.b, c );
+                    if constexpr ( STAGED ) end = !path_continue_staged ( sf, throughput, bounce, p.bounces, pd, wi ); else
                     end = !path_continue<KINDS> ( sf, wo, throughput, bounce, p.bounces, pd, wi );
                     if ( !end ) { ro = surface_origin ( sf, h.point ); rd = wi; }
                     const uint32_t tri = scene_raycast_triangle<COUNT, MODE, ray_start_masks_for ( COUNT, MODE, KINDS )> ( T, shadow_ray, c, pend.expected );
@@ -676,6 +678,7 @@
                     Ray ray_a; V3 b_d;
                     const MisPending pend = mis_prepare<COUNT, KINDS, MODE> ( T, sf, h.point, wo, throughput, bounce, rs.b, c, ray_a, b_d );
                     const V3 next_o = surface_origin ( sf, h.point );
+                    if constexpr ( STAGED ) { pd = path_draw<COUNT> ( azimuth_table<MODE> ( T.sc ), rs.b, c ); end = !path_continue_staged ( sf, throughput, bounce, p.bounces, pd, wi ); } else
                     end = !path_continue<COUNT, KINDS> ( T.sc, sf, wo, throughput, bounce, p.bounces, rs.b, c, wi, sp );
                     if ( !end ) { ro = next_o; rd = wi; }
                     const uint32_t tri_a = scene_raycast_triangle<COUNT, MODE, ray_start_masks_for ( COUNT, MODE, KINDS )> ( T, ray_a, c, pend.expected );
@@ -687,6 +690,7 @@
                 lo_add ( integrate<INTEGRATOR, COUNT, MODE, KINDS> ( T, ray, sf, h.point, wo, throughput, bounce, rs.b, c ) );
                 if ( !pre_draw ) pd = path_draw<COUNT> ( azimuth_table<MODE> ( T.sc ), rs.b, c );
                 if constexpr ( ( KINDS & TERRA_KIND_SAMPLER ) != 0 ) path_apply_sampler ( pd, sp, bounce );
+                if constexpr ( STAGED ) end = !path_continue_staged ( sf, throughput, bounce, p.bounces, pd, wi ); else
                 end = !path_continue<KINDS> ( sf, wo, throughput, bounce, p.bounces, pd, wi );
                 if ( !end ) { ro = surface_origin ( sf, h.point ); rd = wi; }
                 }
diff --git a/terra_amd/csrc/scene_host.cpp b/terra_amd/csrc/scene_host.cpp
--- a/terra_amd/csrc/scene_host.cpp
+++ b/terra_amd/csrc/scene_host.cpp
@@ -1346,6 +1346,14 @@
     p.tan_half_fov = ( float ) tan ( ( double ) ( ( cam->fov * 0.0174533f ) / 2 ) );
     p.aspect = ( float ) fb_w / ( float ) fb_h;
     p.inv_fb_w = 1.f / ( float ) fb_w; p.inv_fb_h = 1.f / ( float ) fb_h;
+    p.shade_s1_guarded = terra_camera_stage_limits ( p.aspect, p.tan_half_fov, p.cam_rot ) ? 0u : 1u;
+}
+extern "C" int terra_amd_shade_stage_info ( const TerraCamera* cam, size_t fb_w, size_t fb_h, int* s1_guarded ) {
+    if ( !cam || !s1_guarded || fb_w == 0 || fb_h == 0 ) return fail ( kTerraAmdErrBadArgument, "terra_amd_shade_stage_info: null camera or result, or an empty frame" );
+    DevRenderParams p; memset ( &p, 0, sizeof p );
+    fill_camera ( cam, fb_w, fb_h, p );
+    *s1_guarded = ( int ) p.shade_s1_guarded;
+    return 0;
 }
 
 static int scene_check ( const Scene* s ) {
@@ -2973,6 +2981,22 @@
     return u.finish ( u.ok ? terra_unit_exact_sqrt ( op, da, db, dc, first, count, seed, dh, dp, dm, dr ) : hipSuccess );
 }
 
+extern "C" int terra_amd_unit_shade_stages ( int stage, int drops, const float* rows, uint64_t count, uint32_t* staged, uint32_t* guarded, uint32_t* mask, uint32_t* full_mask, uint32_t* mismatches ) {
+    if ( need_device() ) return kTerraAmdErrNoDevice;
+    if ( stage < 1 || stage > 5 ) return fail ( kTerraAmdErrBadArgument, "shade_stages unit: stage %d is not one of 1 - 5", stage );
+    if ( stage == 4 ) {
+        if ( !mismatches ) return fail ( kTerraAmdErrBadArgument, "shade_stages unit: stage 4 needs a place for the mismatch count" );
+        *mismatches = 0;
+        Unit u; uint32_t* dm = u.inout ( mismatches, 1 );
+        return u.finish ( u.ok ? terra_unit_shade_stages ( 4, 0, nullptr, 0, nullptr, nullptr, nullptr, nullptr, dm ) : hipSuccess );
+    }
+    if ( count > ( 1ull << 24 ) || ( count && ( !rows || !staged || !guarded || !mask || !full_mask ) ) )
+        return fail ( kTerraAmdErrBadArgument, "shade_stages unit: stage %d needs its rows and four output arrays, at most 2^24 rows", stage );
+    const size_t n = ( size_t ) count;
+    Unit u; const float* dr = u.in ( rows, 16 * n ); uint32_t* ds = u.out ( staged, 8 * n ); uint32_t* dg = u.out ( guarded, 8 * n ); uint32_t* dk = u.out ( mask, n ); uint32_t* df = u.out ( full_mask, n );
+    return u.finish ( u.ok ? terra_unit_shade_stages ( stage, drops, dr, count, ds, dg, dk, df, nullptr ) : hipSuccess );
+}
+
 extern "C" int terra_amd_unit_half_outward ( const double* x, int n, int up, uint16_t* out ) {
     if ( n < 0 || ( n && ( !x || !out ) ) ) return fail ( kTerraAmdErrBadArgument, "null array" );
     for ( int i = 0; i < n; ++i ) out[i] = fastbvh::half_outward ( x[i], up != 0 );
diff --git a/terra_amd/csrc/shading_device.h b/terra_amd/csrc/shading_device.h
--- a/terra_amd/csrc/shading_device.h
+++ b/terra_amd/csrc/shading_device.h
@@ -51,7 +51,17 @@
     int   bsdf;
 };
 
-template <int MODE, int KINDS>
+template <bool SHORT> TD int surface_stage ( float nu, float nv, float div, float rdiv, int flag, V3 na, V3 nb, V3 nc, float& u, float& v, V3& normal ) {
+    int ok = 1;
+    const int g = flag & xd_in_range ( nu ) & xd_in_range ( nv );
+    if constexpr ( SHORT ) ok &= g;
+    if ( SHORT || g ) { u = xd_div_short ( nu, div, rdiv ); v = xd_div_short ( nv, div, rdiv ); }
+    else { u = nu / div; v = nv / div; }
+    const float w = 1 - u - v;
+    normal = normalize_site<SHORT> ( ( nc * v + nb * u ) + na * w, ok );
+    return ok;
+}
+template <int MODE, int KINDS, bool STAGED = false>
 TD void surface_init ( const Tracer& T, uint32_t ti, V3 point, Surface& sf, uint32_t& object_out, uint32_t& tri_in_object_out, uint32_t& nattr_out ) {
     float4 t0, t1, t2, p0, p1, p2, p3x;
     if ( MODE == 1 ) {
@@ -75,6 +85,11 @@
         const float d00 = c1.z, d11 = c1.w, d01 = c2.x, div = c2.y;
         const float dp0 = dot ( p, e0 ), dp1 = dot ( p, e1 );
         const float nu = d11 * dp0 - d01 * dp1, nv = d00 * dp1 - d01 * dp0;
+        if constexpr ( STAGED ) {
+            const V3 na = v3 ( p0.x, p0.y, p0.z ), nb = v3 ( p0.w, p1.x, p1.y ), nc = v3 ( p1.z, p1.w, p2.x );
+            if ( __any ( !surface_stage<true> ( nu, nv, div, c2.z, ( int ) __float_as_uint ( c2.w ), na, nb, nc, u, v, sf.normal ) ) )
+                surface_stage<false> ( nu, nv, div, c2.z, ( int ) __float_as_uint ( c2.w ), na, nb, nc, u, v, sf.normal );
+        } else
         if ( ( int ) __float_as_uint ( c2.w ) & xd_in_range ( nu ) & xd_in_range ( nv ) ) { u = xd_div_short ( nu, div, c2.z ); v = xd_div_short ( nv, div, c2.z ); }
         else { u = nu / div; v = nv / div; }
     } else {
@@ -87,7 +102,7 @@
     }
     float w = 1 - u - v;
     V3 na = v3 ( p0.x, p0.y, p0.z ), nb = v3 ( p0.w, p1.x, p1.y ), nc = v3 ( p1.z, p1.w, p2.x );
-    sf.normal = normalize ( ( nc * v + nb * u ) + na * w );
+    if ( !STAGED || ! ( MODE == 1 && T.l_consts ) ) sf.normal = normalize ( ( nc * v + nb * u ) + na * w );
     const DevMaterial& m = T.l_mats[object];
     sf.emissive = v3p ( m.emissive );
     #pragma unroll
@@ -132,7 +147,7 @@
     if ( res.hit ) {
         uint32_t nattr;
         if ( pre ) *pre = path_draw<COUNT> ( azimuth_table<MODE> ( T.sc ), *rb, c );
-        surface_init<MODE, KINDS> ( T, best.tri, res.point, sf, res.object, res.tri_in_object, nattr );
+        surface_init<MODE, KINDS, MASKS && TERRA_SHADE_STAGES != 0> ( T, best.tri, res.point, sf, res.object, res.tri_in_object, nattr );
         if ( MODE >= 2 ) res.tri = T.sc.mats[res.object].first_tri + res.tri_in_object;
         if ( COUNT ) ++c.hits;
         if ( COUNT == 2 ) c.attr_fetches += nattr + 1;
diff --git a/terra_amd/csrc/trace_geometry.h b/terra_amd/csrc/trace_geometry.h
--- a/terra_amd/csrc/trace_geometry.h
+++ b/terra_amd/csrc/trace_geometry.h
@@ -19,6 +19,16 @@
     float fy = sy * p.tan_half_fov;
     V3 d = normalize ( v3 ( fx, fy, 1.f ) );
     return camera_rotate ( p, d );
+}
+
+TD V3 camera_film_normalize ( float fx, float fy ) {
+    const float l = xs_sqrt_short ( fx * fx + fy * fy + 1.f * 1.f ), r = xd_rcp_short_any ( l );
+    return v3 ( xd_div_short_pos ( fx, l, r ), xd_div_short_pos ( fy, l, r ), xd_div_short_pos ( 1.f, l, r ) );
+}
+TD V3 camera_sample_staged ( const DevRenderParams& p, uint32_t px, uint32_t py, float r1, float r2 ) {
+    if ( p.shade_s1_guarded || TERRA_SHADE_DROPS == 0 ) return camera_sample ( p, px, py, r1, r2 );
+    float sx, sy; camera_film ( p, px, py, r1, r2, sx, sy );
+    return camera_rotate ( p, camera_film_normalize ( sx * p.aspect * p.tan_half_fov, sy * p.tan_half_fov ) );
 }
 
 TD void concentric_disk ( float l1, float l2, float& u, float& v ) {
@@ -195,6 +205,9 @@
 #define TERRA_RAY_START_CAMERA 1
 #endif
 TD constexpr bool ray_start_masks_for ( int COUNT, int MODE, int KINDS ) { return TERRA_RAY_START_CAMERA && MODE == 1 && COUNT == 0 && KINDS == 1; }
+template <bool STAGED> TD V3 camera_direction ( const DevRenderParams& p, uint32_t px, uint32_t py, float r1, float r2 ) {
+    if constexpr ( STAGED ) return camera_sample_staged ( p, px, py, r1, r2 ); else return camera_sample ( p, px, py, r1, r2 );
+}
 
 TD void tri_vertices ( float4 t0, float4 t1, float4 t2, V3& a, V3& b, V3& c ) { a = v3 ( t0.x, t0.y, t0.z ); b = v3 ( t1.x, t1.y, t1.z ); c = v3 ( t2.x, t2.y, t2.z ); }
 TD void tri_vertices ( const float4* tris, uint32_t i, V3& a, V3& b, V3& c ) { tri_vertices ( tris[3 * i], tris[3 * i + 1], tris[3 * i + 2], a, b, c ); }
diff --git a/terra_amd/csrc/trace_math.h b/terra_amd/csrc/trace_math.h
--- a/terra_amd/csrc/trace_math.h
+++ b/terra_amd/csrc/trace_math.h
@@ -25,6 +25,10 @@
 TD float length ( V3 a ) { return sqrtf ( length2 ( a ) ); }
 TD V3 normalize_plain ( V3 a ) { float l = sqrtf ( length2 ( a ) ); return v3 ( a.x / l, a.y / l, a.z / l ); }
 TD V3 normalize ( V3 a ) { float l = sqrt_exact ( length2 ( a ) ); V3 r; xd_normalize3 ( a.x, a.y, a.z, l, r.x, r.y, r.z ); return r; }
+template <bool SHORT> TD V3 normalize_site ( V3 a, int& ok ) {
+    const float l2 = length2 ( a ), l = xs_site_sqrt<SHORT> ( l2, xs_in_range ( l2 ), ok );
+    V3 r; xd_site_normalize3<SHORT> ( a.x, a.y, a.z, l, r.x, r.y, r.z, ok ); return r;
+}
 TD float sel_min ( float a, float b ) { return a < b ? a : b; }
 TD float sel_max ( float a, float b ) { return a > b ? a : b; }
 TD float pick ( V3 a, int i ) { return i == 0 ? a.x : ( i == 1 ? a.y : a.z ); }
@@ -60,6 +64,12 @@
     const float k = sqrt_exact ( a * a + n.z * n.z );
     return basis_of ( v3 ( ( c ? n.z : 0.f ) * k, ( c ? 0.f : -n.z ) * k, ( c ? -n.x : n.y ) * k ), n );
 }
+template <bool SHORT> TD Basis make_basis_site ( V3 n, int& ok ) {
+    const bool c = fabsf ( n.x ) > fabsf ( n.y );
+    const float a = c ? n.x : n.y;
+    const float kk = a * a + n.z * n.z, k = xs_site_sqrt<SHORT> ( kk, xs_in_range ( kk ), ok );
+    return basis_of ( v3 ( ( c ? n.z : 0.f ) * k, ( c ? 0.f : -n.z ) * k, ( c ? -n.x : n.y ) * k ), n );
+}
 
 struct Ray { V3 o, d, inv; };
 TD Ray make_ray ( V3 o, V3 d ) { Ray r; r.o = o; r.d = d; rcp3_exact ( d.x, d.y, d.z, r.inv.x, r.inv.y, r.inv.z ); return r; }
@@ -70,6 +80,28 @@
     else { r.inv.x = 1.f / d.x; r.inv.y = 1.f / d.y; r.inv.z = 1.f / d.z; }
     return r;
 }
+#ifndef TERRA_SHADE_STAGES
+#define TERRA_SHADE_STAGES 1
+#endif
+#ifndef TERRA_SHADE_DROPS
+#define TERRA_SHADE_DROPS 1
+#endif
+template <bool SHORT, bool DROPS> TD int ray_stage ( V3 o, V3 d, Ray& r ) {
+    r.o = o; r.d = d;
+    const int ok = DROPS ? xd_rcp_unit_ok ( d.x ) & xd_rcp_unit_ok ( d.y ) & xd_rcp_unit_ok ( d.z ) : xd_rcp_ok ( d.x ) & xd_rcp_ok ( d.y ) & xd_rcp_ok ( d.z );
+    if ( SHORT || ok ) { r.inv.x = xd_rcp_short ( d.x ); r.inv.y = xd_rcp_short ( d.y ); r.inv.z = xd_rcp_short ( d.z ); }
+    else { r.inv.x = 1.f / d.x; r.inv.y = 1.f / d.y; r.inv.z = 1.f / d.z; }
+    return ok;
+}
+TD Ray make_ray_staged ( V3 o, V3 d, bool& guarded, uint32_t s1_guarded ) {
+    Ray r;
+    if ( s1_guarded ) return make_ray_guarded ( o, d, guarded );
+    if constexpr ( TERRA_SHADE_STAGES != 0 ) {
+        guarded = ray_stage<true, TERRA_SHADE_DROPS != 0> ( o, d, r ) != 0;
+        if ( __any ( !guarded ) ) r = make_ray_guarded ( o, d, guarded );
+    } else guarded = ray_stage<false, TERRA_SHADE_DROPS != 0> ( o, d, r ) != 0;
+    return r;
+}
 
 struct RayState { float shearx, sheary, scalez; int ix, iy, iz; };
 TD V3 permuted ( V3 a, const RayState& s ) { return v3 ( pick ( a, s.ix ), pick ( a, s.iy ), pick ( a, s.iz ) ); }
diff --git a/terra_amd/csrc/unit_kernels.hip b/terra_amd/csrc/unit_kernels.hip
--- a/terra_amd/csrc/unit_kernels.hip
+++ b/terra_amd/csrc/unit_kernels.hip
@@ -537,3 +537,94 @@
     hipLaunchKernelGGL ( k_azimuth24, dim3 ( ( 1u << 24 ) / 256u ), dim3 ( 256 ), 0, 0, table, computed, mismatches );
     return hipGetLastError();
 }
+
+template <int STAGE, bool DROPS>
+__global__ __launch_bounds__ ( 256 ) void k_shade_stages ( const float* rows, unsigned long long n, uint32_t* staged, uint32_t* guarded, uint32_t* mask, uint32_t* full_mask ) {
+    const unsigned long long i = blockIdx.x * 256ull + threadIdx.x;
+    if ( i >= n ) return;
+    const float* q = rows + 16 * i;
+    float s[8] = { 0.f, 0.f, 0.f, 0.f, 0.f, 0.f, 0.f, 0.f }, g[8] = { 0.f, 0.f, 0.f, 0.f, 0.f, 0.f, 0.f, 0.f };
+    int ok = 0, full = 0;
+    if constexpr ( STAGE == 1 ) {
+        const V3 o = v3 ( 0, 0, 0 ), d = v3p ( q );
+        Ray a, b, f; bool gd;
+        ok = ray_stage<true, DROPS> ( o, d, a ); full = ray_stage<true, false> ( o, d, f );
+        if ( __any ( !ok ) ) a = make_ray_guarded ( o, d, gd );
+        b = make_ray_guarded ( o, d, gd );
+        s[0] = a.inv.x; s[1] = a.inv.y; s[2] = a.inv.z; g[0] = b.inv.x; g[1] = b.inv.y; g[2] = b.inv.z;
+    } else if constexpr ( STAGE == 5 ) {
+        const V3 a = camera_film_normalize ( q[0], q[1] ), b = normalize_plain ( v3 ( q[0], q[1], 1.f ) );
+        ok = 1; full = 1;
+        s[0] = a.x; s[1] = a.y; s[2] = a.z; g[0] = b.x; g[1] = b.y; g[2] = b.z;
+    } else if constexpr ( STAGE == 2 ) {
+        const float nu = q[0], nv = q[1], div = q[2], rdiv = rcp_exact ( div ); const int flag = xd_rcp_ok ( div );
+        const V3 na = v3p ( q + 3 ), nb = v3p ( q + 6 ), nc = v3p ( q + 9 );
+        V3 ns, ng;
+        ok = surface_stage<true> ( nu, nv, div, rdiv, flag, na, nb, nc, s[0], s[1], ns ); full = ok;
+        if ( __any ( !ok ) ) surface_stage<false> ( nu, nv, div, rdiv, flag, na, nb, nc, s[0], s[1], ns );
+        surface_stage<false> ( nu, nv, div, rdiv, flag, na, nb, nc, g[0], g[1], ng );
+        s[2] = ns.x; s[3] = ns.y; s[4] = ns.z; g[2] = ng.x; g[3] = ng.y; g[4] = ng.z;
+    } else {
+        const V3 nrm = v3p ( q ), albedo = v3p ( q + 3 ), tp = v3p ( q + 6 );
+        const uint32_t k0 = __float_as_uint ( q[9] ) & 0xffffffu, k1 = __float_as_uint ( q[10] ) & 0xffffffu;
+        PathDraws d; d.e0 = trng_b_from_bits ( k0 ); d.e1 = trng_b_from_bits ( k1 ); d.e2 = 0.f; d.e3 = q[11]; d.az = azimuth_fetch_index ( nullptr, k1 );
+        V3 ws, ts, wg, tg, wf, tf; bool gs, gg, gf;
+        ok = continue_stage<true, DROPS> ( nrm, albedo, tp, d, ws, ts, gs ); full = continue_stage<true, false> ( nrm, albedo, tp, d, wf, tf, gf );
+        if ( __any ( !ok ) ) continue_stage<false, false> ( nrm, albedo, tp, d, ws, ts, gs );
+        Surface sf; sf.normal = nrm; sf.emissive = v3 ( 0, 0, 0 ); sf.attr[0] = albedo; sf.attr[1] = sf.attr[2] = sf.attr[3] = v3 ( 0, 0, 0 ); sf.ior = 1.f; sf.bsdf = kDevBsdfDiffuse;
+        uint32_t bounce = 0; tg = tp;
+        gg = path_continue<1> ( sf, v3 ( 0, 0, 1 ), tg, bounce, 1000u, d, wg );
+        {
+            uint32_t bits = 0;
+            const float r = sqrt_exact ( d.e0 ); float sn, cs; azimuth_sincos ( d.az, d.e1, sn, cs );
+            const float om = sel_max ( 0.f, 1 - d.e0 );
+            const V3 local = v3 ( r * cs, sqrt_exact ( om ), r * sn );
+            const float ba = fabsf ( nrm.x ) > fabsf ( nrm.y ) ? nrm.x : nrm.y;
+            const V3 v = basis_apply ( make_basis ( nrm ), local );
+            const float l2 = length2 ( v ), l = sqrt_exact ( l2 );
+            const V3 w = normalize ( v );
+            const float num = sel_max ( 0.f, dot ( nrm, w ) ), pdf = sel_max ( diffuse_pdf ( sf, w ), ( float ) 1e-4 );
+            V3 t = had ( tp, diffuse_eval ( sf ) * rcp_exact ( pdf ) ); t = t * dot ( nrm, w );
+            const float pr = sel_max ( t.x, sel_max ( t.y, t.z ) );
+            bits |= xs_in_range ( d.e0 ) ? 1u : 0u; bits |= xs_in_range ( om ) ? 2u : 0u; bits |= xs_in_range ( ba * ba + nrm.z * nrm.z ) ? 4u : 0u; bits |= xs_in_range ( l2 ) ? 8u : 0u;
+            bits |= ( ( int ) ( l >= 0x1p-60f ) & ( int ) ( l <= 0x1p60f ) & xd_component_ok ( v.x ) & xd_component_ok ( v.y ) & xd_component_ok ( v.z ) ) ? 16u : 0u;
+            bits |= ( __float_as_uint ( l ) & 0x7fffffu ) != 0x7fffffu ? 32u : 0u;
+            bits |= xd_in_range ( num ) ? 64u : 0u; bits |= xd_rcp_ok ( pdf ) ? 128u : 0u;
+            bits |= ( ( ( int ) ( pr >= 0.f ) & ( int ) ( pr <= 0x1p60f ) ) | ( int ) ( d.e3 > pr ) ) ? 256u : 0u;
+            g[7] = __uint_as_float ( bits );
+        }
+        s[0] = ws.x; s[1] = ws.y; s[2] = ws.z; s[3] = ts.x; s[4] = ts.y; s[5] = ts.z; s[6] = gs ? 1.f : 0.f;
+        g[0] = wg.x; g[1] = wg.y; g[2] = wg.z; g[3] = tg.x; g[4] = tg.y; g[5] = tg.z; g[6] = gg ? 1.f : 0.f;
+    }
+    for ( int j = 0; j < 8; ++j ) { staged[8 * i + j] = __float_as_uint ( s[j] ); guarded[8 * i + j] = __float_as_uint ( g[j] ); }
+    mask[i] = ( uint32_t ) ok; full_mask[i] = ( uint32_t ) full;
+}
+__global__ __launch_bounds__ ( 256 ) void k_variate_roots ( uint32_t* mismatches ) {
+    const uint32_t k = blockIdx.x * 256u + threadIdx.x;
+    const float e = trng_b_from_bits ( k ), om = sel_max ( 0.f, 1 - e );
+    const bool admitted = xs_variate_ok ( e ) != 0;
+    uint32_t bad = 0;
+    if ( admitted && __float_as_uint ( xs_sqrt_short ( e ) ) != __float_as_uint ( sqrt_exact ( e ) ) ) ++bad;
+    if ( !admitted && k != 0u ) ++bad;
+    if ( __float_as_uint ( xs_sqrt_short ( om ) ) != __float_as_uint ( sqrt_exact ( om ) ) ) ++bad;
+    const float d = __uint_as_float ( ( ( 67u + k % 121u ) << 23 ) | 0x7fffffu | ( ( k / 121u ) & 1u ) << 31 );
+    if ( k < 242u && __float_as_uint ( xd_rcp_all_ones ( d ) ) != __float_as_uint ( 1.f / d ) ) ++bad;
+    const float l = __builtin_fabsf ( d );
+    const uint32_t h = ( uint32_t ) xd_hash ( k );
+    const float x = __uint_as_float ( ( __float_as_uint ( l ) & 0x7f800000u ) - ( ( ( h >> 23 ) % 21u ) << 23 ) | ( h & 0x807fffffu ) );
+    if ( xd_in_range ( x ) && __float_as_uint ( xd_div_short_pos ( x, l, xd_rcp_short_any ( l ) ) ) != __float_as_uint ( x / l ) ) ++bad;
+    if ( bad ) atomicAdd ( mismatches, bad );
+}
+hipError_t terra_unit_shade_stages ( int stage, int drops, const float* rows, uint64_t n, uint32_t* staged, uint32_t* guarded, uint32_t* mask, uint32_t* full_mask, uint32_t* mismatches ) {
+    const dim3 grid ( ( unsigned ) ( ( n + 255 ) / 256 ) ), block ( 256 );
+#define SS_CASE(S, D) hipLaunchKernelGGL ( ( k_shade_stages<S, D> ), grid, block, 0, 0, rows, ( unsigned long long ) n, staged, guarded, mask, full_mask )
+    if ( stage == 4 ) hipLaunchKernelGGL ( k_variate_roots, dim3 ( ( 1u << 24 ) / 256u ), dim3 ( 256 ), 0, 0, mismatches );
+    else if ( n == 0 ) return hipSuccess;
+    else if ( stage == 1 ) { if ( drops ) SS_CASE ( 1, true ); else SS_CASE ( 1, false ); }
+    else if ( stage == 5 ) SS_CASE ( 5, false );
+    else if ( stage == 2 ) SS_CASE ( 2, false );
+    else if ( stage == 3 ) { if ( drops ) SS_CASE ( 3, true ); else SS_CASE ( 3, false ); }
+    else return hipErrorInvalidValue;
+#undef SS_CASE
+    return hipGetLastError();
+}
```
